# dimforge/salva

Hardware: AMD Instinct MI355X
Metric: particle-steps/sec (3D DFSPH) (higher is better)
Workload: dtype f32

## Files before the change

### salva_amd/csrc/device_types.h

```cpp
#pragma once
#include <hip/hip_runtime.h>

#include <cstdint>

#include "sph_math.h"

namespace salva {

struct TileGrid {
    int ox, oy, oz;
    int ntx, nty, ntz;
    uint32_t mx, my, mz;
    const uint32_t* cell_start;
};

struct TileAcc {
    uint64_t s;
    uint64_t sb;
    uint32_t nsl;
    uint32_t nonempty;
    uint32_t max_s, max_sb, max_nsl;
    uint32_t max_sum;
    uint32_t max_raw;
    uint32_t wsl;
    uint32_t ntiny;
    uint32_t heavy;
    uint32_t nlight;
    __host__ __device__ TileAcc operator+(const TileAcc& o) const {
        return TileAcc{s + o.s, sb + o.sb, nsl + o.nsl, nonempty + o.nonempty, max_s > o.max_s ? max_s : o.max_s,
                       max_sb > o.max_sb ? max_sb : o.max_sb, max_nsl > o.max_nsl ? max_nsl : o.max_nsl,
                       max_sum > o.max_sum ? max_sum : o.max_sum, max_raw > o.max_raw ? max_raw : o.max_raw, wsl + o.wsl, ntiny + o.ntiny, heavy + o.heavy, nlight + o.nlight};
    }
};

struct alignas(16) SolveCtl {
    uint32_t done;
    uint32_t iters;
    float err;
    uint32_t seq;
    float tol;
    uint32_t min_iter;
    uint32_t mode;
    uint32_t pad;
};
static_assert(sizeof(SolveCtl) == 32, "SolveCtl: two 16-byte halves");

struct TileListStats { uint32_t sum_ff, sum_fb, max_ff, max_fb, own_ff, own_fb, ref_s, ref_sb; };

struct PrePub { int32_t on, chained; int32_t bbox[6]; };

struct StepCtx {
    SphConsts sc;
    uint32_t xcd;

    uint32_t n;
    float4* posm;
    float4* vel;
    float4* dv;
    float4* acc;
    float4* w;
    float4* normal;
    uint32_t* model;
    uint32_t* perm;
    const uint32_t* gtag;
    float* rho;
    float* alpha;
    float* kappa;
    float* kappa2;
    float* rho_star;
    float* aii;
    float4* dii;
    float4* dijpj;
    float4* posmr;
    float4* iisph_q;
    float4* iisph_pr;
    uint32_t* nff;
    uint32_t* nfb;
    uint32_t* nbr_ff;
    uint32_t* nbr_fb;
    uint32_t* slice_near;
    uint32_t cap_ff, cap_fb;
    const TileAcc* tile_off;
    const uint32_t* halo_src;
    const uint32_t* bhalo_src;
    uint32_t halo_stride;
    uint32_t bhalo_stride;
    uint32_t ntiles;
    uint32_t split_s;
    const uint32_t* tile_ids;
    const uint4* slot_desc;
    const uint4* slot_info;
    const uint32_t* tile_rank;
    const uint32_t* slot_order;
    uint32_t slot_base;
    uint32_t ntiny;
    uint32_t nlight;
    uint32_t nlaunch;
    uint32_t spec;
    uint32_t halo_cap, bhalo_cap;
    uint32_t nslices_cap;
    uint64_t halo_len, bhalo_len;
    TileGrid gf;
    const uint32_t* stale_keys;

    uint32_t nb;
    float4* bposv;
    float4* bvel;
    uint32_t* bperm;
    float4* bforce;
    unsigned long long* bforce_fx;
    float bforce_scale;
    const uint8_t* bwants;
    TileGrid gb;

    uint32_t nmodels, nbmodels;
    const float* rho0_tab;
    float rho0_single;
    float mass_uniform;
    uint32_t* tile_mass_bits;
    uint32_t* tile_massb_bits;
    uint2* tile_masscd_bits;
    uint32_t* nffb;
    uint32_t* nffc;
    uint32_t two_mass;
    uint32_t nmass;
    uint64_t cmask;
    float class_mass[4];
    uint32_t bvel_zero;
    const uint8_t* ff_ok;
    const uint8_t* fb_ok;
    const uint8_t* bb_ok;

    float* partials;
    int spec_k;
    uint32_t spec_external;
    SolveCtl* spec_ring;
    SolveCtl* spec_pub;
    const uint32_t* model_counts;
    float4* w2;
    uint32_t* flags;
    uint32_t min_neighbors_for_divergence;
    int32_t phase, ghost_lo_cx, ghost_hi_cx;
    const SolveCtl* ctl;
    const uint32_t* gate;
    uint32_t gate_stage;
#ifdef SALVA_HIP_DIAG
    unsigned long long* dbg;
#endif
};

constexpr uint32_t MASS_SLOTS = 64;

struct Readback {
    float err;
    uint32_t flags;
    int32_t bbox[6];
    int32_t bbbox[6];
    TileAcc tile_total;
    uint64_t ncontacts_bb;
    uint64_t ncontacts_ff, ncontacts_fb;
    uint32_t max_cnt_ff, max_cnt_fb;
    uint32_t dcs_count;
    uint32_t cfl_max_bits;
    uint64_t ncontacts_own_ff, ncontacts_own_fb;
    uint32_t mass_mm[2];
    uint32_t pad2_[2];
    uint32_t chain_ok, chain_stage;
    uint32_t solve[2][4];
    uint32_t pre_ok;
    uint32_t max_ref[3];
};
// ... 7 lines not shown
```

### salva_amd/csrc/dfsph.hip

```cpp
#include <climits>

#include "bbox.h"
#include "kernels.h"
#include "tile.h"

namespace SALVA_KNS {
using namespace salva;

unsigned num_blocks(uint32_t n) { return div_up(n, BLOCK); }

}
#include "pairs.h"
namespace SALVA_KNS {
using namespace salva;

static inline bool plane_layouts(const StepCtx& c) { return c.mass_uniform > 0.0f || c.two_mass != 0u; }

#ifndef SALVA_DA_IISPH_WAVES
#define SALVA_DA_IISPH_WAVES 6
#endif
template <bool IISPH>
__global__ __launch_bounds__(TILE_MAX_THREADS, IISPH ? SALVA_DA_IISPH_WAVES : 1) void k_density_alpha(StepCtx c, float dt) {
    lds_base_check();
    Tile t;
    t.setup(c);
    if (t.empty()) return;
    struct Own { float4 pi; uint32_t mi, cnt; ListRegs lh; };
    auto load_own = [&](uint32_t i, uint32_t gs) { return Own{c.posm[i], c.model[i], c.nff[i], list_regs(c, gs)}; };
    uint32_t i0, gs0;
    t.first_own(i0, gs0);
    const Own own0 = load_own(i0, gs0);
    const float4* Lp = nullptr;
    t.stage(c, static_cast<const float4*>(c.posm), Lp);
    const float4* Bp = nullptr;
    t.stage_boundary(c, Bp);
    Tile::staged_barrier();
    t.for_own_pre(own0, load_own, [&](const Own& o, uint32_t i, uint32_t gs, bool active) {
        const uint32_t nqu = slice_list_dwords(o.cnt, active);
        const float4 pi = o.pi;
        float rho = 0.0f, gsx = 0.0f, gsy = 0.0f, gsz = 0.0f, sq = 0.0f;
        uint32_t nnear = 0;
        if (active) {
            f2 rw = {0.0f, 0.0f}, ax = {0.0f, 0.0f}, ay = {0.0f, 0.0f}, az = {0.0f, 0.0f}, s2 = {0.0f, 0.0f};
            const f2 tiny = {1.0e-30f, 1.0e-30f};
            for_each_ff2<true, false, true>(c, gs, nqu, o.lh, [&](uint32_t off) { return lds_ld16(off); }, [&](const float4& A, const float4& B) { SALVA_PAIR_MATH
                const f2 dx = {pi.x - A.x, pi.x - B.x}, dy = {pi.y - A.y, pi.y - B.y}, dz = {pi.z - A.z, pi.z - B.z};
                f2 r2 = dz * dz + tiny;
                r2 = dy * dy + r2;
                r2 = dx * dx + r2;
                const bool za = r2.x <= c.sc.tiny_r2, zb = r2.y <= c.sc.tiny_r2;
                nnear += (za ? 1u : 0u) + (zb ? 1u : 0u);
                const KernelWG2 k = kernel_wg2(r2, c.sc);
                const f2 m = {A.w, B.w};
                f2 wm = k.w * m;
                wm.x = za ? 0.0f : wm.x; wm.y = zb ? 0.0f : wm.y;
                rw += wm;
                const f2 gm = k.g * m;
                ax += dx * gm; ay += dy * gm; az += dz * gm;
                if (!IISPH) s2 += (gm * gm) * r2;
                else s2 += (k.g * gm) * r2;
            });
            const uint32_t npad = 2u * nqu - o.cnt;
            rho = (rw.x + rw.y) * c.sc.wscale + pi.w * c.sc.wnorm;
            gsx = (ax.x + ax.y) * c.sc.gscale; gsy = (ay.x + ay.y) * c.sc.gscale; gsz = (az.x + az.y) * c.sc.gscale;
            sq = (s2.x + s2.y) * (c.sc.gscale * c.sc.gscale);
            nnear -= npad;
        }
#ifdef SALVA_OTHER_KERNELS
        const bool any_near = __builtin_amdgcn_ballot_w64(active && nnear > 1u) != 0ull || (c.sc.kd | c.sc.kg) != 0;
#else
        const bool any_near = __builtin_amdgcn_ballot_w64(active && nnear > 1u) != 0ull;
#endif
        if (any_near && active) {
            rho = gsx = gsy = gsz = sq = 0.0f;
            for_each_ff(c, i, gs, [&](uint32_t s) { SALVA_PAIR_MATH
                const float4 pj = lds_ld16(s << 4);
                const float dx = pi.x - pj.x, dy = pi.y - pj.y, dz = pi.z - pj.z;
                const KernelEval e = kernel_eval(dx * dx + dy * dy + dz * dz, c.sc);
                rho += pj.w * e.w;
                const float gm = e.g * pj.w;
                const float gx = dx * gm, gy = dy * gm, gz = dz * gm;
                if (!IISPH) sq += gx * gx + gy * gy + gz * gz;
// ... 234 lines not shown
template <uint32_t DS>
__global__ __launch_bounds__(TILE_MAX_THREADS) void k_divergence(StepCtx c) {
    const SolveCtl* const rec = solve_record(c);
    if (rec && rec->done) return;
    const float4* const win = rec ? solve_w_in(c, rec) : c.w;
    lds_base_check();
    Tile t;
    t.setup(c);
    if (t.skipped()) return;
    if (t.empty()) { TileErr::zero(c, t.slot); return; }
    struct Own { float4 pi, wi; float alpha; uint32_t mi, cnt, cntb, near; ListRegs lh; };
    auto load_own = [&](uint32_t i, uint32_t gs) {
        return Own{c.posm[i], win[i], c.alpha[i], c.model[i], c.nff[i], c.nb ? c.nfb[i] : 0u, c.slice_near[gs], list_regs(c, gs)};
    };
    uint32_t i0, gs0;
    t.first_own(i0, gs0);
    const Own own0 = load_own(i0, gs0);
    const uint32_t dist = pw_dist<DS>(c, t);
    const float4* Bp = nullptr;
    const float4* Bv = nullptr;
    t.stage_pw(c, static_cast<const float4*>(c.posm), win, dist, Bp, Bv, false);
    TileErr E;
    E.init(carve_errtab(t), c);
    Tile::staged_barrier();
    t.for_own_pre(own0, load_own, [&](const Own& o, uint32_t i, uint32_t gs, bool active) {
        const uint32_t nqu = slice_list_dwords(o.cnt, active);
        const bool near = slice_is_near(c, o.near);
        float err = 0.0f;
        uint32_t mi = 0;
        if (active) {
            mi = o.mi;
            const float rho0 = rho0_of(c, mi);
            float div = 0.0f;
            if (o.cnt + o.cntb >= c.min_neighbors_for_divergence) {
                const float4 pi = o.pi, wi = o.wi;
                div += near ? pair_sum_velocity_divergence_exact(c, i, gs, pi, wi, dist)
                            : pair_sum_velocity_divergence(c, gs, nqu, o.lh, pi, wi, dist);
                for_each_fb(c, t, i, gs, [&](uint32_t s) { SALVA_PAIR_MATH
                    const float4 pj = Bp[s];
                    const float dx = pi.x - pj.x, dy = pi.y - pj.y, dz = pi.z - pj.z;
                    const float g = kernel_grad(dx * dx + dy * dy + dz * dz, c.sc);
                    div += (wi.x * dx + wi.y * dy + wi.z * dz) * g * (pj.w * rho0);
                });
                div = fmaxf(div, 0.0f);
            }
            c.kappa[i] = div * o.alpha;
            err = div / rho0;
        }
        E.add(c, err, mi, active && !is_ghost(c, i));
    });
    E.finish(c, t.slot);
}
#define SALVA_P3_BOUNDS(DS) __launch_bounds__(TILE_MAX_THREADS, (DS) == P3_DS_THREE ? 6 : 5)
#ifndef SALVA_EVAL_POST
#define SALVA_EVAL_POST false
#endif
template <uint32_t DS, int TWO>
__device__ __forceinline__ void k_divergence_p3_body(StepCtx c) {
    const SolveCtl* const rec = solve_record(c);
    if (rec && rec->done) return;
    const float4* const win = rec ? solve_w_in(c, rec) : c.w;
    lds_base_check();
    Tile t;
    t.setup(c);
    if (t.skipped()) return;
    if (t.empty()) { TileErr::zero(c, t.slot); return; }
    constexpr bool POST = TWO || SALVA_EVAL_POST;
    struct Own { float px, py, pz, ux, uy, uz, alpha; uint32_t mi, cnt, cntb, nb2, near; ListRegs lh; };
    auto load_own = [&](uint32_t i, uint32_t gs) {
        const float4 p = c.posm[i], u = win[i];
        return Own{p.x, p.y, p.z, u.x, u.y, u.z, POST ? 0.0f : c.alpha[i], POST ? 0u : c.model[i], c.nff[i], c.nb ? c.nfb[i] : 0u,
                   (TWO && t.massb != 0.0f) ? c.nffb[i] : 0u, c.slice_near[gs], list_regs(c, gs)};
    };
    uint32_t i0, gs0;
    t.first_own(i0, gs0);
    const Own own0 = load_own(i0, gs0);
    const uint32_t dist8 = p3_dist8<DS>(t);
    t.stage_p3(c, static_cast<const float4*>(c.posm), win, dist8);
    const float4* Bp = nullptr;
    t.stage_boundary(c, Bp);
    TileErrC E;
    E.init(reinterpret_cast<float*>(t.pool + t.pool_used), c);
    Tile::staged_barrier();
    t.for_own_pre(own0, load_own, [&](const Own& o, uint32_t i, uint32_t gs, bool active) {
        const uint32_t nqu = slice_list_dwords(o.cnt, active);
        const bool near = slice_is_near(c, o.near);
        float err = 0.0f;
        uint32_t mi = 0;
        if (active) {
            mi = POST ? c.model[i] : o.mi;
            const float rho0 = rho0_of(c, mi);
            float div = 0.0f;
            if (o.cnt + o.cntb >= c.min_neighbors_for_divergence) {
                const float4 pi = make_float4(o.px, o.py, o.pz, 0.0f), wi = make_float4(o.ux, o.uy, o.uz, 0.0f);
                if ((TWO && t.massb != 0.0f) && !near) {
                    div += pair_sum_velocity_divergence_p3_two(c, gs, nqu, o.lh, pi, wi, dist8, o.cnt - o.nb2, t.mass, t.massb);
                } else {
                    div += near ? pair_sum_velocity_divergence_exact_p3(c, i, gs, pi, wi, dist8, t.mass)
                                : pair_sum_velocity_divergence_p3(c, gs, nqu, o.lh, pi, wi, dist8, t.mass);
                    if ((TWO && t.massb != 0.0f) && o.nb2)
                        div += (t.massb - t.mass) * pair_tail_velocity_divergence_p3(c, gs, o.cnt - o.nb2, o.cnt, pi, wi, dist8);
                }
                if (TWO == 2 && t.massc != 0.0f) {
                    const uint32_t cd = c.nffc[i], l2 = cd & 0xffffu, l3 = cd >> 16;
                    if (l2) div += (t.massc - t.massb) * pair_tail_velocity_divergence_p3(c, gs, o.cnt - l3 - l2, o.cnt - l3, pi, wi, dist8);
                    if (l3) div += (t.massd - t.massb) * pair_tail_velocity_divergence_p3(c, gs, o.cnt - l3, o.cnt, pi, wi, dist8);
                }
                for_each_fb(c, t, i, gs, [&](uint32_t s) { SALVA_PAIR_MATH
                    const float4 pj = Bp[s];
                    const float dx = pi.x - pj.x, dy = pi.y - pj.y, dz = pi.z - pj.z;
                    const float g = kernel_grad(dx * dx + dy * dy + dz * dz, c.sc);
                    div += (wi.x * dx + wi.y * dy + wi.z * dz) * g * (pj.w * rho0);
                });
                div = fmaxf(div, 0.0f);
            }
            c.kappa[i] = div * (POST ? c.alpha[i] : o.alpha);
            err = div / rho0;
        }
        E.add(c, err, mi, active && !is_ghost(c, i));
    });
    E.finish(c, t.slot);
}
template <uint32_t DS>
__global__ SALVA_P3_BOUNDS(DS) void k_divergence_p3(StepCtx c) { k_divergence_p3_body<DS, 0>(c); }
template <uint32_t DS>
__global__ SALVA_P3_BOUNDS(DS) void k_divergence_p3_two(StepCtx c) { k_divergence_p3_body<DS, 1>(c); }
template <uint32_t DS>
__global__ SALVA_P3_BOUNDS(DS) void k_divergence_p3_multi(StepCtx c) { k_divergence_p3_body<DS, 2>(c); }
void launch_divergence(const StepCtx& c, const TileLds& L, hipStream_t s) {
    SALVA_OK_DISPATCH(launch_divergence, c, L, s);
    if (plane_layouts(c)) {
        const uint32_t ds = pick_ds_p3(L.max_halo_fluid, L.ds_level);
        if (c.two_mass && c.nmass > 2u) SALVA_LAUNCH_P3(k_divergence_p3_multi, ds, c, L, p3_bytes(L, ds, c.nmodels, false), s, c);
        else if (c.two_mass) SALVA_LAUNCH_P3(k_divergence_p3_two, ds, c, L, p3_bytes(L, ds, c.nmodels, false), s, c);
        else SALVA_LAUNCH_P3(k_divergence_p3, ds, c, L, p3_bytes(L, ds, c.nmodels, false), s, c);
        return;
    }
    const uint32_t ds = pick_ds(pw_slots(L), L.ds_level);
    SALVA_LAUNCH_FIXED(k_divergence, ds, c, L, pw_bytes(L, ds, true), s, c);
}

template <uint32_t DS>
__global__ __launch_bounds__(TILE_MAX_THREADS) void k_divergence_apply(StepCtx c, float inv_dt_prev) {
    const SolveCtl* const rec = solve_record(c);
    const bool was_done = rec && rec->done;
    const float4* const win = rec ? solve_w_in(c, rec) : c.w;
    float4* const wout = c.spec_k >= 0 ? ((win == c.w) ? c.w2 : c.w) : c.w;
    lds_base_check();
    if (c.spec_k >= 0 && !c.spec_external && blockIdx.x == 0 && c.slot_base == 0u) {
        spec_decide(c, reinterpret_cast<float*>(tile_smem));
        __syncthreads();
    }
    if (was_done) return;
    Tile t;
    t.setup(c);
    if (t.empty()) return;
    struct Own { float4 pi, wi; float ki; uint32_t cnt, near; ListRegs lh; };
    auto load_own = [&](uint32_t i, uint32_t gs) {
        return Own{c.posm[i], win[i], c.kappa[i], c.nff[i], c.slice_near[gs], list_regs(c, gs)};
    };
    uint32_t i0, gs0;
    t.first_own(i0, gs0);
    const Own own0 = load_own(i0, gs0);
    const uint32_t dist = pk_dist<DS>(c, t);
    const float4* Bp = nullptr;
    const float4* Bv = nullptr;
    t.stage_pk(c, static_cast<const float4*>(c.posm), static_cast<const float*>(c.kappa), dist, Bp, Bv);
    Tile::staged_barrier();
    t.for_own_pre(own0, load_own, [&](const Own& o, uint32_t i, uint32_t gs, bool active) {
        const uint32_t nqu = slice_list_dwords(o.cnt, active);
        const bool near = slice_is_near(c, o.near);
        if (!active) return;
        const float4 pi = o.pi;
        const uint32_t mi = __float_as_uint(o.wi.w);
        const float rho0 = rho0_of(c, mi);
        const float ki = o.ki;
        float4 d = o.wi;
        float sx, sy, sz;
        if (near) pair_sum_gradient_exact(c, i, gs, pi, dist, [&](float kj) { return ki + kj; }, sx, sy, sz);
        else pair_sum_gradient(c, gs, nqu, o.lh, pi, dist, [&](float ka, float kb) { return f2{ki + ka, ki + kb}; }, sx, sy, sz);
        d.x -= sx; d.y -= sy; d.z -= sz;
        for_each_fb(c, t, i, gs, [&](uint32_t s) { SALVA_PAIR_MATH
            const float4 pj = Bp[s];
            const float dx = pi.x - pj.x, dy = pi.y - pj.y, dz = pi.z - pj.z;
            const float g = kernel_grad(dx * dx + dy * dy + dz * dz, c.sc);
            const float coeff = -ki * pj.w * rho0 * g;
            const float ex = dx * coeff, ey = dy * coeff, ez = dz * coeff;
            d.x += ex; d.y += ey; d.z += ez;
            if (c.bforce && !is_ghost(c, i)) {
                const float fs = -inv_dt_prev * pi.w;
                apply_boundary_force(c, boundary_sorted_of_slot(c, t, s), __float_as_uint(Bv[s].w), ex * fs, ey * fs, ez * fs);
            }
        });
        wout[i] = d;
    });
}
#ifndef SALVA_P2_WAVES
#define SALVA_P2_WAVES 6
#endif
#define SALVA_P2_BOUNDS(DS) __launch_bounds__(TILE_MAX_THREADS, (DS) == P2_DS_THREE ? SALVA_P2_WAVES : 5)
template <uint32_t DS, int TWO>
__device__ __forceinline__ void k_divergence_apply_p2_body(StepCtx c, float inv_dt_prev) {
    const SolveCtl* const rec = solve_record(c);
    const bool was_done = rec && rec->done;
    const float4* const win = rec ? solve_w_in(c, rec) : c.w;
    float4* const wout = c.spec_k >= 0 ? ((win == c.w) ? c.w2 : c.w) : c.w;
    lds_base_check();
    if (c.spec_k >= 0 && !c.spec_external && blockIdx.x == 0 && c.slot_base == 0u) {
        spec_decide(c, reinterpret_cast<float*>(tile_smem));
        __syncthreads();
    }
    if (was_done) return;
    Tile t;
    t.setup(c);
    if (t.empty()) return;
    struct Own { float px, py, pz, ki; uint32_t cnt, nb2, near; ListRegs lh; };
    auto load_own = [&](uint32_t i, uint32_t gs) {
        const float4 p = c.posm[i];
        return Own{p.x, p.y, p.z, c.kappa[i], c.nff[i], (TWO && t.massb != 0.0f) ? c.nffb[i] : 0u, c.slice_near[gs], list_regs(c, gs)};
    };
    uint32_t i0, gs0;
    t.first_own(i0, gs0);
    const Own own0 = load_own(i0, gs0);
    const uint32_t dist8 = p2_dist8<DS>(t);
    t.stage_p2(c, static_cast<const float4*>(c.posm), static_cast<const float*>(c.kappa), dist8);
    Tile::staged_barrier();
    t.for_own_pre(own0, load_own, [&](const Own& o, uint32_t i, uint32_t gs, bool active) {
        const uint32_t nqu = slice_list_dwords(o.cnt, active);
        const bool near = slice_is_near(c, o.near);
        if (!active) return;
        const float4 pi = make_float4(o.px, o.py, o.pz, 0.0f);
        const float ki = o.ki;
        float sx, sy, sz;
        if ((TWO && t.massb != 0.0f) && !near) {
            pair_sum_gradient_p2_two(c, gs, nqu, o.lh, pi, dist8, o.cnt - o.nb2, t.mass, t.massb, [&](float ka, float kb) { return f2{ki + ka, ki + kb}; }, sx, sy, sz);
        } else {
            if (near) pair_sum_gradient_exact_p2(c, i, gs, pi, dist8, t.mass, [&](float kj) { return ki + kj; }, sx, sy, sz);
            else pair_sum_gradient_p2(c, gs, nqu, o.lh, pi, dist8, t.mass, [&](float ka, float kb) { return f2{ki + ka, ki + kb}; }, sx, sy, sz);
            if ((TWO && t.massb != 0.0f) && o.nb2) {
                float bx, by, bz;
                pair_tail_gradient_p2(c, gs, o.cnt - o.nb2, o.cnt, pi, dist8, [&](float kj) { return ki + kj; }, bx, by, bz);
                const float dm = t.massb - t.mass;
                sx += dm * bx; sy += dm * by; sz += dm * bz;
            }
        }
        if (TWO == 2 && t.massc != 0.0f) {
            const uint32_t cd = c.nffc[i], l2 = cd & 0xffffu, l3 = cd >> 16;
            float bx, by, bz;
            if (l2) {
                pair_tail_gradient_p2(c, gs, o.cnt - l3 - l2, o.cnt - l3, pi, dist8, [&](float kj) { return ki + kj; }, bx, by, bz);
                const float dm = t.massc - t.massb;
                sx += dm * bx; sy += dm * by; sz += dm * bz;
            }
            if (l3) {
                pair_tail_gradient_p2(c, gs, o.cnt - l3, o.cnt, pi, dist8, [&](float kj) { return ki + kj; }, bx, by, bz);
                const float dm = t.massd - t.massb;
                sx += dm * bx; sy += dm * by; sz += dm * bz;
            }
        }
        float4 d = win[i];
        const uint32_t mi = __float_as_uint(d.w);
        const float rho0 = rho0_of(c, mi);
        d.x -= sx; d.y -= sy; d.z -= sz;
        for_each_fb(c, t, i, gs, [&](uint32_t s) { SALVA_PAIR_MATH
            const float4 pj = p2_boundary_pos(t, s, dist8);
            const float dx = pi.x - pj.x, dy = pi.y - pj.y, dz = pi.z - pj.z;
            const float g = kernel_grad(dx * dx + dy * dy + dz * dz, c.sc);
            const float coeff = -ki * pj.w * rho0 * g;
            const float ex = dx * coeff, ey = dy * coeff, ez = dz * coeff;
            d.x += ex; d.y += ey; d.z += ez;
            if (c.bforce && !is_ghost(c, i)) {
                const float fs = -inv_dt_prev * c.posm[i].w;
                const uint32_t jb = boundary_sorted_of_slot(c, t, s);
                apply_boundary_force(c, jb, __float_as_uint(c.bvel[jb].w), ex * fs, ey * fs, ez * fs);
            }
        });
        wout[i] = d;
    });
}
template <uint32_t DS>
__global__ SALVA_P2_BOUNDS(DS) void k_divergence_apply_p2(StepCtx c, float inv_dt_prev) { k_divergence_apply_p2_body<DS, 0>(c, inv_dt_prev); }
template <uint32_t DS>
__global__ SALVA_P2_BOUNDS(DS) void k_divergence_apply_p2_two(StepCtx c, float inv_dt_prev) { k_divergence_apply_p2_body<DS, 1>(c, inv_dt_prev); }
template <uint32_t DS>
__global__ SALVA_P2_BOUNDS(DS) void k_divergence_apply_p2_multi(StepCtx c, float inv_dt_prev) { k_divergence_apply_p2_body<DS, 2>(c, inv_dt_prev); }
void launch_divergence_apply(const StepCtx& c, const TileLds& L, float inv_dt_prev, hipStream_t s) {
    SALVA_OK_DISPATCH(launch_divergence_apply, c, L, inv_dt_prev, s);
    if (plane_layouts(c)) {
        const uint32_t ds = pick_ds_p2(L.raw_slots(), L.ds_level);
        if (c.two_mass && c.nmass > 2u) SALVA_LAUNCH_P2(k_divergence_apply_p2_multi, ds, c, L, p2_bytes(L, ds), s, c, inv_dt_prev);
        else if (c.two_mass) SALVA_LAUNCH_P2(k_divergence_apply_p2_two, ds, c, L, p2_bytes(L, ds), s, c, inv_dt_prev);
        else SALVA_LAUNCH_P2(k_divergence_apply_p2, ds, c, L, p2_bytes(L, ds), s, c, inv_dt_prev);
        return;
    }
    const uint32_t ds = pick_ds(pk_slots(L), L.ds_level);
    SALVA_LAUNCH_FIXED(k_divergence_apply, ds, c, L, pk_bytes(L, ds), s, c, inv_dt_prev);
}

__global__ __launch_bounds__(BLOCK) void k_finish_divergence(StepCtx c, float gx, float gy, float gz, int acc_has_user) {
    const uint32_t i = blockIdx.x * BLOCK + threadIdx.x;
    if (i >= c.n || gate_closed(c)) return;
    const float4 wi = c.w[i];
    const float4 v = c.vel[i];
    const float4 d = c.dv[i];
    c.vel[i] = make_float4(wi.x, wi.y, wi.z, v.w);
    c.dv[i] = make_float4(0.0f, 0.0f, 0.0f, d.w);
    float4 a = make_float4(0.0f, 0.0f, 0.0f, 0.0f);
    if (acc_has_user) a = c.acc[i];
    c.acc[i] = make_float4(a.x + gx, a.y + gy, a.z + gz, 0.0f);
}
void launch_finish_divergence(const StepCtx& c, float gx, float gy, float gz, bool acc_has_user, hipStream_t s) {
    if (c.n) k_finish_divergence<<<num_blocks(c.n), BLOCK, 0, s>>>(c, gx, gy, gz, acc_has_user ? 1 : 0);
}

__global__ __launch_bounds__(BLOCK) void k_integrate(StepCtx c, float dt) {
    const uint32_t i = blockIdx.x * BLOCK + threadIdx.x;
    if (i >= c.n || gate_closed(c)) return;
    const float4 a = c.acc[i];
    float4 d = c.dv[i];
    d.x += a.x * dt; d.y += a.y * dt; d.z += a.z * dt;
    c.dv[i] = d;
    c.acc[i] = make_float4(0.0f, 0.0f, 0.0f, 0.0f);
    const float4 v = c.vel[i];
    c.w[i] = make_float4(v.x + d.x, v.y + d.y, v.z + d.z, __uint_as_float(c.model[i]));
}
void launch_integrate(const StepCtx& c, float dt, hipStream_t s) {
    if (c.n) k_integrate<<<num_blocks(c.n), BLOCK, 0, s>>>(c, dt);
}

#ifdef SALVA_HIP_DIAG
#define SALVA_DIAG_STAMP(name) const unsigned long long name = __builtin_readcyclecounter()
#else
#define SALVA_DIAG_STAMP(name)
#endif
template <uint32_t DS>
__global__ __launch_bounds__(TILE_MAX_THREADS) void k_pred_density(StepCtx c, float dt) {
    if (c.ctl && c.ctl->done) return;
    lds_base_check();
    SALVA_DIAG_STAMP(T0);
    Tile t;
    t.setup(c);
    if (t.skipped()) return;
    if (t.empty()) { TileErr::zero(c, t.slot); return; }
    SALVA_DIAG_STAMP(T1);
    struct Own { float4 pi, wi; float rho, alpha; uint32_t mi, cnt, near; ListRegs lh; };
    auto load_own = [&](uint32_t i, uint32_t gs) {
        return Own{c.posm[i], c.w[i], c.rho[i], c.alpha[i], c.model[i], c.nff[i], c.slice_near[gs], list_regs(c, gs)};
    };
    uint32_t i0, gs0;
    t.first_own(i0, gs0);
    const Own own0 = load_own(i0, gs0);
    const uint32_t dist = pw_dist<DS>(c, t);
    const float4* Bp = nullptr;
    const float4* Bv = nullptr;
    t.stage_pw(c, static_cast<const float4*>(c.posm), static_cast<const float4*>(c.w), dist, Bp, Bv, true);
    TileErr E;
    E.init(carve_errtab(t), c);
    SALVA_DIAG_STAMP(T2);
    Tile::staged_barrier();
    SALVA_DIAG_STAMP(T3);
    t.for_own_pre(own0, load_own, [&](const Own& o, uint32_t i, uint32_t gs, bool active) {
// ... 437 lines not shown
```

### salva_amd/csrc/pairs.h

```cpp
#pragma once
#include <cstdlib>

#include "tile.h"

namespace salva {

struct RecPW { float4 p, w; };
struct RecPK { float4 p; float k; };

__device__ __forceinline__ float rho0_of(const StepCtx& c, uint32_t model) {
    return (c.nmodels == 1) ? c.rho0_single : c.rho0_tab[model];
}

template <uint32_t DS>
__device__ __forceinline__ uint32_t pw_dist(const StepCtx& c, const Tile& t) { return DS ? DS * 16u : (t.stage_cap(c) + t.SB) * 16u; }
template <uint32_t DS>
__device__ __forceinline__ uint32_t pk_dist(const StepCtx& c, const Tile& t) { return DS ? DS * 16u : (t.stage_cap(c) + 2u * t.SB) * 16u; }

__device__ __forceinline__ RecPW load_pw(uint32_t o, uint32_t dist) {
    RecPW r{lds_ld16(o), lds_ld16(o + dist)};
    asm volatile("" ::"v"(r.w.w));
    return r;
}
__device__ __forceinline__ RecPK load_pk(uint32_t o, uint32_t dist) { return RecPK{lds_ld16(o), lds_ld4((o >> 2) + dist)}; }

template <bool AHEAD = true>
__device__ __forceinline__ float pair_sum_velocity_divergence(const StepCtx& c, uint32_t gs, uint32_t nqu, const ListRegs& lh,
                                                              const float4& pi, const float4& wi, uint32_t dist) {
    f2 acc2 = {0.0f, 0.0f};
    const f2 tiny = {1.0e-30f, 1.0e-30f};
    for_each_ff2<AHEAD, false, true>(c, gs, nqu, lh, [&](uint32_t o) { return load_pw(o, dist);
    }, [&](const RecPW& A, const RecPW& B) { SALVA_PAIR_MATH
        const f2 dx = {pi.x - A.p.x, pi.x - B.p.x}, dy = {pi.y - A.p.y, pi.y - B.p.y}, dz = {pi.z - A.p.z, pi.z - B.p.z};
        f2 r2 = dz * dz + tiny;
        r2 = dy * dy + r2;
        r2 = dx * dx + r2;
        const f2 g = kernel_gfac2(r2, c.sc);
        const f2 ux = {wi.x - A.w.x, wi.x - B.w.x}, uy = {wi.y - A.w.y, wi.y - B.w.y}, uz = {wi.z - A.w.z, wi.z - B.w.z};
        const f2 gm = {g.x * A.p.w, g.y * B.p.w};
        acc2 += (ux * dx + uy * dy + uz * dz) * gm;
    });
    return (acc2.x + acc2.y) * c.sc.gscale;
}
__device__ __forceinline__ float pair_sum_velocity_divergence_exact(const StepCtx& c, uint32_t i, uint32_t gs, const float4& pi,
                                                                    const float4& wi, uint32_t dist) {
    float acc = 0.0f;
    for_each_ff(c, i, gs, [&](uint32_t s) { SALVA_PAIR_MATH
        const RecPW A = load_pw(s << 4, dist);
        const float dx = pi.x - A.p.x, dy = pi.y - A.p.y, dz = pi.z - A.p.z;
        const float g = kernel_grad(dx * dx + dy * dy + dz * dz, c.sc);
        acc += ((wi.x - A.w.x) * dx + (wi.y - A.w.y) * dy + (wi.z - A.w.z) * dz) * g * A.p.w;
    });
    return acc;
}
struct RecP3 { lds_v2f xy, zu, vw; };
template <uint32_t DS>
__device__ __forceinline__ uint32_t p3_dist8(const Tile& t) { return DS ? DS * 8u : ((t.S * 8u + 15u) & ~15u); }
template <uint32_t DS>
__device__ __forceinline__ uint32_t p2_dist8(const Tile& t) { return DS ? DS * 8u : (((t.S + t.SB) * 8u + 15u) & ~15u); }
__device__ __forceinline__ RecP3 load_p3(uint32_t o, uint32_t dist8) { return RecP3{lds_ld8(o), lds_ld8(o + dist8), lds_ld8(o + 2u * dist8)}; }
template <bool AHEAD = true>
__device__ __forceinline__ float pair_sum_velocity_divergence_p3(const StepCtx& c, uint32_t gs, uint32_t nqu, const ListRegs& lh,
                                                                 const float4& pi, const float4& wi, uint32_t dist8, float mass) {
    f2 acc2 = {0.0f, 0.0f};
    const f2 tiny = {1.0e-30f, 1.0e-30f};
    for_each_ff2<AHEAD, false, 2>(c, gs, nqu, lh, [&](uint32_t o) { return load_p3(o, dist8); }, [&](const RecP3& A, const RecP3& B) { SALVA_PAIR_MATH
        const f2 dx = {pi.x - A.xy.x, pi.x - B.xy.x}, dy = {pi.y - A.xy.y, pi.y - B.xy.y}, dz = {pi.z - A.zu.x, pi.z - B.zu.x};
        f2 r2 = dz * dz + tiny;
        r2 = dy * dy + r2;
        r2 = dx * dx + r2;
        const f2 g = kernel_gfac2(r2, c.sc);
        const f2 ux = {wi.x - A.zu.y, wi.x - B.zu.y}, uy = {wi.y - A.vw.x, wi.y - B.vw.x}, uz = {wi.z - A.vw.y, wi.z - B.vw.y};
        acc2 += (ux * dx + uy * dy + uz * dz) * g;
    });
    return (acc2.x + acc2.y) * c.sc.gscale * mass;
}
__device__ __forceinline__ float pair_sum_velocity_divergence_p3_two(const StepCtx& c, uint32_t gs, uint32_t nqu, const ListRegs& lh, const float4& pi,
                                                                     const float4& wi, uint32_t dist8, uint32_t na, float ma, float mb) {
    f2 acc2 = {0.0f, 0.0f};
    const f2 tiny = {1.0e-30f, 1.0e-30f};
    for_each_ff2_indexed<2>(c, gs, nqu, lh, [&](uint32_t o) { return load_p3(o, dist8); }, [&](const RecP3& A, const RecP3& B, uint32_t q) { SALVA_PAIR_MATH
        const f2 dx = {pi.x - A.xy.x, pi.x - B.xy.x}, dy = {pi.y - A.xy.y, pi.y - B.xy.y}, dz = {pi.z - A.zu.x, pi.z - B.zu.x};
        f2 r2 = dz * dz + tiny;
        r2 = dy * dy + r2;
        r2 = dx * dx + r2;
        const f2 g = kernel_gfac2(r2, c.sc);
        const f2 ux = {wi.x - A.zu.y, wi.x - B.zu.y}, uy = {wi.y - A.vw.x, wi.y - B.vw.x}, uz = {wi.z - A.vw.y, wi.z - B.vw.y};
        const f2 m = {2u * q < na ? ma : mb, 2u * q + 1u < na ? ma : mb};
        acc2 += (ux * dx + uy * dy + uz * dz) * (g * m);
    });
    return (acc2.x + acc2.y) * c.sc.gscale;
}
__device__ __forceinline__ float pair_sum_velocity_divergence_exact_p3(const StepCtx& c, uint32_t i, uint32_t gs, const float4& pi,
                                                                       const float4& wi, uint32_t dist8, float mass) {
    float acc = 0.0f;
    for_each_ff(c, i, gs, [&](uint32_t s) { SALVA_PAIR_MATH
        const RecP3 A = load_p3(s << 3, dist8);
        const float dx = pi.x - A.xy.x, dy = pi.y - A.xy.y, dz = pi.z - A.zu.x;
        const float g = kernel_grad(dx * dx + dy * dy + dz * dz, c.sc);
        acc += ((wi.x - A.zu.y) * dx + (wi.y - A.vw.x) * dy + (wi.z - A.vw.y) * dz) * g;
    });
    return acc * mass;
}
template <typename F>
__device__ __forceinline__ void for_each_ff_range(const StepCtx& c, uint32_t gs, uint32_t first, uint32_t cnt, F&& f) {
    const uint32_t* __restrict__ p = c.nbr_ff + (size_t)gs * c.cap_ff * WAVE + 4u * (threadIdx.x & (WAVE - 1));
    for (uint32_t e = first; e < cnt; ++e) {
        const uint32_t d = p[ellq(e >> 1)];
        f((e & 1u) ? (d >> 16) : (d & 0xffffu));
    }
}
__device__ __forceinline__ float pair_tail_velocity_divergence_p3(const StepCtx& c, uint32_t gs, uint32_t first, uint32_t cnt, const float4& pi,
                                                                  const float4& wi, uint32_t dist8) {
    float acc = 0.0f;
    for_each_ff_range(c, gs, first, cnt, [&](uint32_t s) { SALVA_PAIR_MATH
        const RecP3 A = load_p3(s << 3, dist8);
        const float dx = pi.x - A.xy.x, dy = pi.y - A.xy.y, dz = pi.z - A.zu.x;
        const float g = kernel_grad(dx * dx + dy * dy + dz * dz, c.sc);
        acc += ((wi.x - A.zu.y) * dx + (wi.y - A.vw.x) * dy + (wi.z - A.vw.y) * dz) * g;
    });
    return acc;
}
struct RecP2 { lds_v2f xy, zk; };
__device__ __forceinline__ RecP2 load_p2(uint32_t o, uint32_t dist8) { return RecP2{lds_ld8(o), lds_ld8(o + dist8)}; }
#ifndef SALVA_P2_NARROW
#define SALVA_P2_NARROW false
#endif
template <typename K2>
__device__ __forceinline__ void pair_sum_gradient_p2(const StepCtx& c, uint32_t gs, uint32_t nqu, const ListRegs& lh, const float4& pi,
                                                     uint32_t dist8, float mass, K2&& kij2, float& sx, float& sy, float& sz) {
    f2 ax = {0.0f, 0.0f}, ay = {0.0f, 0.0f}, az = {0.0f, 0.0f};
    const f2 tiny = {1.0e-30f, 1.0e-30f};
    for_each_ff2<true, false, 2, SALVA_P2_NARROW>(c, gs, nqu, lh, [&](uint32_t o) { return load_p2(o, dist8); }, [&](const RecP2& A, const RecP2& B) { SALVA_PAIR_MATH
        const f2 dx = {pi.x - A.xy.x, pi.x - B.xy.x}, dy = {pi.y - A.xy.y, pi.y - B.xy.y}, dz = {pi.z - A.zk.x, pi.z - B.zk.x};
        f2 r2 = dz * dz + tiny;
        r2 = dy * dy + r2;
        r2 = dx * dx + r2;
        const f2 g = kernel_gfac2(r2, c.sc);
        const f2 coeff = kij2(A.zk.y, B.zk.y) * g;
        ax += dx * coeff; ay += dy * coeff; az += dz * coeff;
    });
    const float f = c.sc.gscale * mass;
    sx = (ax.x + ax.y) * f; sy = (ay.x + ay.y) * f; sz = (az.x + az.y) * f;
}
template <typename K2>
__device__ __forceinline__ void pair_sum_gradient_p2_two(const StepCtx& c, uint32_t gs, uint32_t nqu, const ListRegs& lh, const float4& pi,
                                                         uint32_t dist8, uint32_t na, float ma, float mb, K2&& kij2, float& sx, float& sy, float& sz) {
    f2 ax = {0.0f, 0.0f}, ay = {0.0f, 0.0f}, az = {0.0f, 0.0f};
    const f2 tiny = {1.0e-30f, 1.0e-30f};
    for_each_ff2_indexed<2>(c, gs, nqu, lh, [&](uint32_t o) { return load_p2(o, dist8); }, [&](const RecP2& A, const RecP2& B, uint32_t q) { SALVA_PAIR_MATH
        const f2 dx = {pi.x - A.xy.x, pi.x - B.xy.x}, dy = {pi.y - A.xy.y, pi.y - B.xy.y}, dz = {pi.z - A.zk.x, pi.z - B.zk.x};
        f2 r2 = dz * dz + tiny;
        r2 = dy * dy + r2;
        r2 = dx * dx + r2;
        const f2 g = kernel_gfac2(r2, c.sc);
        const f2 m = {2u * q < na ? ma : mb, 2u * q + 1u < na ? ma : mb};
        const f2 coeff = kij2(A.zk.y, B.zk.y) * (g * m);
        ax += dx * coeff; ay += dy * coeff; az += dz * coeff;
    });
    sx = (ax.x + ax.y) * c.sc.gscale; sy = (ay.x + ay.y) * c.sc.gscale; sz = (az.x + az.y) * c.sc.gscale;
}
template <typename K1>
__device__ __forceinline__ void pair_sum_gradient_exact_p2(const StepCtx& c, uint32_t i, uint32_t gs, const float4& pi, uint32_t dist8,
                                                           float mass, K1&& kij1, float& sx, float& sy, float& sz) {
    float ax = 0.0f, ay = 0.0f, az = 0.0f;
    for_each_ff(c, i, gs, [&](uint32_t s) { SALVA_PAIR_MATH
        const RecP2 A = load_p2(s << 3, dist8);
        const float dx = pi.x - A.xy.x, dy = pi.y - A.xy.y, dz = pi.z - A.zk.x;
        const float coeff = kij1(A.zk.y) * kernel_grad(dx * dx + dy * dy + dz * dz, c.sc);
        ax += dx * coeff; ay += dy * coeff; az += dz * coeff;
    });
    sx = ax * mass; sy = ay * mass; sz = az * mass;
}
template <typename K1>
__device__ __forceinline__ void pair_tail_gradient_p2(const StepCtx& c, uint32_t gs, uint32_t first, uint32_t cnt, const float4& pi, uint32_t dist8,
                                                      K1&& kij1, float& sx, float& sy, float& sz) {
    float ax = 0.0f, ay = 0.0f, az = 0.0f;
    for_each_ff_range(c, gs, first, cnt, [&](uint32_t s) { SALVA_PAIR_MATH
        const RecP2 A = load_p2(s << 3, dist8);
        const float dx = pi.x - A.xy.x, dy = pi.y - A.xy.y, dz = pi.z - A.zk.x;
        const float coeff = kij1(A.zk.y) * kernel_grad(dx * dx + dy * dy + dz * dz, c.sc);
        ax += dx * coeff; ay += dy * coeff; az += dz * coeff;
    });
    sx = ax; sy = ay; sz = az;
}
__device__ __forceinline__ float4 p2_boundary_pos(const Tile& t, uint32_t s, uint32_t dist8) {
    const uint32_t o = (t.S + s) * 8u;
    const lds_v2f xy = lds_ld8(o), zv = lds_ld8(o + dist8);
    return make_float4(xy.x, xy.y, zv.x, zv.y);
}
static inline uint32_t p2_bytes(const TileLds& L, uint32_t ds) {
    const uint32_t n = L.raw_slots();
    const uint32_t dist8 = ds ? ds * 8u : ((n * 8u + 15u) & ~15u);
    return dist8 + n * 8u + 32u;
}

template <typename K2>
__device__ __forceinline__ void pair_sum_gradient(const StepCtx& c, uint32_t gs, uint32_t nqu, const ListRegs& lh, const float4& pi,
                                                  uint32_t dist, K2&& kij2, float& sx, float& sy, float& sz) {
    f2 ax = {0.0f, 0.0f}, ay = {0.0f, 0.0f}, az = {0.0f, 0.0f};
    const f2 tiny = {1.0e-30f, 1.0e-30f};
    for_each_ff2<true, false, true>(c, gs, nqu, lh, [&](uint32_t o) { return load_pk(o, dist); }, [&](const RecPK& A, const RecPK& B) { SALVA_PAIR_MATH
        const f2 dx = {pi.x - A.p.x, pi.x - B.p.x}, dy = {pi.y - A.p.y, pi.y - B.p.y}, dz = {pi.z - A.p.z, pi.z - B.p.z};
        f2 r2 = dz * dz + tiny;
        r2 = dy * dy + r2;
        r2 = dx * dx + r2;
        const f2 g = kernel_gfac2(r2, c.sc);
        const f2 km = kij2(A.k, B.k) * f2{A.p.w, B.p.w};
        const f2 coeff = km * g;
        ax += dx * coeff; ay += dy * coeff; az += dz * coeff;
    });
    sx = (ax.x + ax.y) * c.sc.gscale; sy = (ay.x + ay.y) * c.sc.gscale; sz = (az.x + az.y) * c.sc.gscale;
}
template <typename K1>
__device__ __forceinline__ void pair_sum_gradient_exact(const StepCtx& c, uint32_t i, uint32_t gs, const float4& pi, uint32_t dist,
                                                        K1&& kij1, float& sx, float& sy, float& sz) {
    float ax = 0.0f, ay = 0.0f, az = 0.0f;
    for_each_ff(c, i, gs, [&](uint32_t s) { SALVA_PAIR_MATH
        const RecPK A = load_pk(s << 4, dist);
        const float dx = pi.x - A.p.x, dy = pi.y - A.p.y, dz = pi.z - A.p.z;
        const float coeff = kij1(A.k) * A.p.w * kernel_grad(dx * dx + dy * dy + dz * dz, c.sc);
        ax += dx * coeff; ay += dy * coeff; az += dz * coeff;
    });
    sx = ax; sy = ay; sz = az;
}
__device__ __forceinline__ bool slice_is_near(const StepCtx& c, uint32_t near_word) {
#ifdef SALVA_OTHER_KERNELS
    return (__builtin_amdgcn_readfirstlane((int)near_word) | c.sc.kg) != 0;
#else
    return __builtin_amdgcn_readfirstlane((int)near_word) != 0;
#endif
}
__device__ __forceinline__ float (*carve_errtab(Tile& t))[MAX_MODELS] {
    return reinterpret_cast<float (*)[MAX_MODELS]>(t.carve<float>(TILE_MAX_WAVES * MAX_MODELS));
}

#define SALVA_LAUNCH_FIXED(kernel, DSV, c, L, lds, s, ...)                                                         \
    do {                                                                                                           \
        if ((DSV) == FIXED_DS_SMALL) SALVA_LAUNCH_TILE_3(kernel<FIXED_DS_SMALL>, kernel<FIXED_DS_SMALL>, FIXED_DS_SMALL, kernel<0u>, c, L, lds, s, __VA_ARGS__); \
        else if ((DSV) == FIXED_DS_LARGE) SALVA_LAUNCH_TILE_3(kernel<FIXED_DS_LARGE>, kernel<FIXED_DS_SMALL>, FIXED_DS_SMALL, kernel<0u>, c, L, lds, s, __VA_ARGS__); \
        else SALVA_LAUNCH_TILE_3(kernel<0u>, kernel<FIXED_DS_SMALL>, FIXED_DS_SMALL, kernel<0u>, c, L, lds, s, __VA_ARGS__); \
    } while (0)
static inline uint32_t pick_ds(uint32_t slots_needed, uint32_t level) {
    const uint32_t ds[3] = {FIXED_DS_SMALL, FIXED_DS_LARGE, 0u};
    uint32_t k = slots_needed <= FIXED_DS_SMALL ? 0u : (slots_needed <= FIXED_DS_LARGE ? 1u : 2u);
    k += level;
    return ds[k < 2u ? k : 2u];
}
static inline uint32_t pw_slots(const TileLds& L) { return L.sum_slots(); }
static inline uint32_t pw_bytes(const TileLds& L, uint32_t ds, bool errtab) {
    return (ds ? 2u * ds : 2u * pw_slots(L)) * 16u + (errtab ? TILE_ERR_BYTES : 0u) + 32u;
}
static inline uint32_t pick_ds_p3(uint32_t s, uint32_t level) {
    const uint32_t ds[4] = {P3_DS_THREE, P3_DS_TWO, P3_DS_ONE, 0u};
    uint32_t k = s <= P3_DS_THREE ? 0u : (s <= P3_DS_TWO ? 1u : (s <= P3_DS_ONE ? 2u : 3u));
    k += level;
    return ds[k < 3u ? k : 3u];
}
static inline uint32_t p3_bytes(const TileLds& L, uint32_t ds, uint32_t nmodels, bool with_bv) {
    const uint32_t dist8 = ds ? ds * 8u : ((L.max_halo_fluid * 8u + 15u) & ~15u);
    const uint32_t bb = with_bv ? 32u : 16u;
    const uint32_t by_maxima = ((L.max_halo_fluid * 8u + 15u) & ~15u) + bb * L.max_halo_boundary;
    const uint32_t by_raw = ((L.raw_slots() * 8u + 15u) & ~15u) + (bb - 8u) * L.max_halo_boundary;
    static const uint32_t pad = getenv("SALVA_HIP_P3_PAD") ? (uint32_t)atoi(getenv("SALVA_HIP_P3_PAD")) : 0u;
    return 2u * dist8 + (by_raw < by_maxima ? by_raw : by_maxima) + ((TILE_MAX_WAVES * nmodels * 4u + 15u) & ~15u) + 32u + pad;
}
static inline uint32_t pick_ds_p2(uint32_t n, uint32_t level) {
    const uint32_t ds[4] = {P2_DS_THREE, P3_DS_TWO, P3_DS_ONE, 0u};
    uint32_t k = n <= P2_DS_THREE ? 0u : (n <= P3_DS_TWO ? 1u : (n <= P3_DS_ONE ? 2u : 3u));
    k += level;
    return ds[k < 3u ? k : 3u];
}
#define SALVA_LAUNCH_P3(kernel, DSV, c, L, lds, s, ...)                                                                                          \
    do {                                                                                                                                         \
        if ((DSV) == P3_DS_THREE) SALVA_LAUNCH_TILE_3(kernel<P3_DS_THREE>, kernel<P3_DS_THREE>, P3_DS_THREE, kernel<0u>, c, L, lds, s, __VA_ARGS__); \
        else if ((DSV) == P3_DS_TWO) SALVA_LAUNCH_TILE_3(kernel<P3_DS_TWO>, kernel<P3_DS_THREE>, P3_DS_THREE, kernel<0u>, c, L, lds, s, __VA_ARGS__); \
        else if ((DSV) == P3_DS_ONE) SALVA_LAUNCH_TILE_3(kernel<P3_DS_ONE>, kernel<P3_DS_THREE>, P3_DS_THREE, kernel<0u>, c, L, lds, s, __VA_ARGS__); \
        else SALVA_LAUNCH_TILE_3(kernel<0u>, kernel<P3_DS_THREE>, P3_DS_THREE, kernel<0u>, c, L, lds, s, __VA_ARGS__);                             \
    } while (0)
#define SALVA_LAUNCH_P2(kernel, DSV, c, L, lds, s, ...)                                                                                          \
    do {                                                                                                                                         \
        if ((DSV) == P2_DS_THREE) SALVA_LAUNCH_TILE_3(kernel<P2_DS_THREE>, kernel<P2_DS_THREE>, P2_DS_THREE, kernel<0u>, c, L, lds, s, __VA_ARGS__); \
        else if ((DSV) == P3_DS_TWO) SALVA_LAUNCH_TILE_3(kernel<P3_DS_TWO>, kernel<P2_DS_THREE>, P2_DS_THREE, kernel<0u>, c, L, lds, s, __VA_ARGS__); \
        else if ((DSV) == P3_DS_ONE) SALVA_LAUNCH_TILE_3(kernel<P3_DS_ONE>, kernel<P2_DS_THREE>, P2_DS_THREE, kernel<0u>, c, L, lds, s, __VA_ARGS__); \
        else SALVA_LAUNCH_TILE_3(kernel<0u>, kernel<P2_DS_THREE>, P2_DS_THREE, kernel<0u>, c, L, lds, s, __VA_ARGS__);                             \
    } while (0)
static inline uint32_t pk_slots(const TileLds& L) { return L.sum_slots() + L.max_halo_boundary; }
static inline uint32_t pk_bytes(const TileLds& L, uint32_t ds) {
    return (ds ? ds : pk_slots(L)) * 16u + ((L.max_halo_fluid + 63u) & ~63u) * 4u + 32u;
}


}
```

### salva_amd/csrc/tile.h

```cpp
#pragma once
#include "common.h"
#include "device_types.h"

namespace salva {

#ifndef SALVA_TX
#define SALVA_TX 4
#endif
constexpr int TX = SALVA_TX, TY = 4, TZ = 4;
constexpr int TCELLS = TX * TY * TZ;
constexpr int HX = TX + 2, HY = TY + 2, HZ = TZ + 2;
constexpr int HCELLS = HX * HY * HZ;
constexpr int TILE_MAX_WAVES = 12;
constexpr int TILE_MAX_THREADS = TILE_MAX_WAVES * WAVE;

__host__ __device__ inline int floor_div(int a, int b) { return (a >= 0) ? a / b : -((-a + b - 1) / b); }

__host__ __device__ inline uint32_t ellq(uint32_t q) { return (q >> 2) * (4u * (uint32_t)WAVE) + (q & 3u); }

constexpr uint32_t TILE_TABLE_BYTES = 4 * (2 * (HCELLS + 1) + 2 * HCELLS) + 16;

struct TileLds {
    uint32_t max_halo_fluid = 0, max_halo_boundary = 0, threads = 4 * WAVE;
    uint32_t max_sum = 0;
    uint32_t max_raw = 0;
    uint32_t ds_level = 0;
    uint32_t raw_slots() const { return max_raw ? max_raw : max_halo_fluid + max_halo_boundary; }
    uint32_t sum_slots() const {
        const uint32_t worst = ((max_halo_fluid + 63u) & ~63u) + max_halo_boundary;
        return max_sum ? (max_sum < worst ? max_sum : worst) : worst;
    }
    uint32_t bytes(uint32_t bytes_per_fluid_slot, uint32_t bytes_per_boundary_slot, uint32_t narrays,
                   bool with_cell_tables = false) const {
        const uint32_t separate = ((max_halo_fluid + 63u) & ~63u) * bytes_per_fluid_slot + max_halo_boundary * bytes_per_boundary_slot;
        const uint32_t wide = bytes_per_fluid_slot > bytes_per_boundary_slot ? bytes_per_fluid_slot : bytes_per_boundary_slot;
        const uint32_t joint = sum_slots() * wide;
        return (with_cell_tables ? TILE_TABLE_BYTES : 0u) + (joint < separate ? joint : separate) + 16u * narrays;
    }
};

#ifndef SALVA_FIXED_DS_SMALL
#define SALVA_FIXED_DS_SMALL 2448
#endif
constexpr uint32_t FIXED_DS_SMALL = SALVA_FIXED_DS_SMALL, FIXED_DS_LARGE = 3984;
#ifndef SALVA_P3_DS3
#define SALVA_P3_DS3 2080
#endif
constexpr uint32_t P3_DS_THREE = SALVA_P3_DS3, P3_DS_TWO = 3360, P3_DS_ONE = 4064;
#ifndef SALVA_P2_DS3
#define SALVA_P2_DS3 2464
#endif
constexpr uint32_t P2_DS_THREE = SALVA_P2_DS3;
static_assert((P3_DS_THREE % 64 == 32 && P3_DS_TWO % 64 == 32 && P3_DS_ONE % 64 == 32 && P2_DS_THREE % 64 == 32) || SALVA_P3_DS3 != 2080 || SALVA_P2_DS3 != 2464,
              "plane distances: odd multiples of 256 bytes");
constexpr uint32_t TILE_PART_SHIFT = 28;
constexpr uint32_t TILE_PART_WHOLE = (uint32_t)(TX - 1) << 2;
__host__ __device__ inline uint32_t tile_part_code(uint32_t ux0, uint32_t len) { return ux0 | ((len - 1u) << 2); }
constexpr uint32_t TILE_SPLIT_S = P3_DS_THREE;
constexpr uint32_t TILE_TINY_S = 192, TILE_TINY_SB = 64, TILE_TINY_THREADS = 64;
constexpr uint32_t TILE_ERR_BYTES = 12u * 32u * 4u;

#ifdef __HIPCC__

void raise_tile_lds_limit(const void* kernel, uint32_t bytes);
template <typename K>
inline void ensure_tile_lds(K kernel, uint32_t bytes) {
    if (bytes > 48u * 1024u) raise_tile_lds_limit(reinterpret_cast<const void*>(kernel), bytes);
}
inline TileLds tile_tiny_lds(const TileLds& L) {
    TileLds t = L;
    t.max_halo_fluid = TILE_TINY_S; t.max_halo_boundary = L.max_halo_boundary ? TILE_TINY_SB : 0u;
    t.max_sum = ((TILE_TINY_S + 63u) & ~63u) + t.max_halo_boundary; t.max_raw = TILE_TINY_S + t.max_halo_boundary;
    t.threads = TILE_TINY_THREADS;
    return t;
}
__host__ __device__ inline bool tile_is_light(uint32_t s, uint32_t sb) {
    return s <= P3_DS_THREE && ((s + 63u) & ~63u) + 2u * sb <= FIXED_DS_SMALL;
}
inline TileLds tile_light_lds(const TileLds& L) {
    TileLds t = L;
    t.max_halo_fluid = L.max_halo_fluid < P3_DS_THREE ? L.max_halo_fluid : P3_DS_THREE;
    t.max_halo_boundary = L.max_halo_boundary < FIXED_DS_SMALL / 2u ? L.max_halo_boundary : FIXED_DS_SMALL / 2u;
    t.max_sum = (L.max_sum && L.max_sum < FIXED_DS_SMALL) ? L.max_sum : FIXED_DS_SMALL;
    t.max_raw = (L.max_raw && L.max_raw < FIXED_DS_SMALL) ? L.max_raw : FIXED_DS_SMALL;
    return t;
}
#define SALVA_LAUNCH_TILE_3(kernel, kernel_light, ds_light, kernel_tiny, c, L, lds, s, ...)         \
    do {                                                                                           \
        if ((c).n && (c).nlaunch) {                                                                \
            if (((c).ntiny == 0u && (c).nlight == 0u) || (c).slot_order == nullptr) {              \
                const uint32_t _lds = (lds);                                                       \
                ::salva::ensure_tile_lds(kernel, _lds);                                            \
                kernel<<<(c).nlaunch, (L).threads, _lds, s>>>(__VA_ARGS__);                        \
            } else {                                                                               \
                const uint32_t _ntiny = (c).ntiny, _nlight = (c).nlight;                           \
                const uint32_t _nfull = (c).nlaunch - _nlight - _ntiny;                            \
                ::salva::StepCtx _c2 = (c);                                                        \
                const ::salva::TileLds _lt = ::salva::tile_tiny_lds(L);                            \
                const ::salva::TileLds _ll = ::salva::tile_light_lds(L);                           \
                const unsigned _thr = (L).threads;                                                 \
                if (_nfull) {                                                                      \
                    const uint32_t _lds = (lds);                                                   \
                    ::salva::ensure_tile_lds(kernel, _lds);                                        \
                    _c2.slot_base = 0u;                                                            \
                    { const ::salva::StepCtx c = _c2; kernel<<<_nfull, _thr, _lds, s>>>(__VA_ARGS__); } \
                }                                                                                  \
                if (_nlight) {                                                                     \
                    _c2.slot_base = _nfull;                                                        \
                    const ::salva::TileLds L = _ll;                                                \
                    const uint32_t ds = (ds_light); (void)ds;                                      \
                    const ::salva::StepCtx c = _c2;                                                \
                    const uint32_t _lds = (lds);                                                   \
                    ::salva::ensure_tile_lds(kernel_light, _lds);                                  \
                    kernel_light<<<_nlight, _thr, _lds, s>>>(__VA_ARGS__);                         \
                }                                                                                  \
                if (_ntiny) {                                                                      \
                    _c2.slot_base = _nfull + _nlight;                                              \
                    const ::salva::TileLds L = _lt;                                                \
                    const uint32_t ds = 0u; (void)ds;                                              \
                    const ::salva::StepCtx c = _c2;                                                \
                    const uint32_t _lds = (lds);                                                   \
                    ::salva::ensure_tile_lds(kernel_tiny, _lds);                                   \
                    kernel_tiny<<<_ntiny, TILE_TINY_THREADS, _lds, s>>>(__VA_ARGS__);              \
                }                                                                                  \
            }                                                                                      \
            SALVA_HIP_CHECK(hipGetLastError());                                                    \
        }                                                                                          \
    } while (0)
#define SALVA_LAUNCH_TILE(kernel, c, L, lds, s, ...) SALVA_LAUNCH_TILE_3(kernel, kernel, 0u, kernel, c, L, lds, s, __VA_ARGS__)

__device__ __forceinline__ uint32_t tile_key_m(const TileGrid& g, int cx, int cy, int cz, bool& inside, uint32_t mx, uint32_t my, uint32_t mz) {
    const uint32_t ix = ((uint32_t)cx - (uint32_t)g.ox) & mx, iy = ((uint32_t)cy - (uint32_t)g.oy) & my, iz = ((uint32_t)cz - (uint32_t)g.oz) & mz;
    inside = ix < (uint32_t)(g.ntx * TX) && iy < (uint32_t)(g.nty * TY) && iz < (uint32_t)(g.ntz * TZ);
    const uint32_t tile = ((ix / TX) * (uint32_t)g.nty + (iy / TY)) * (uint32_t)g.ntz + (iz / TZ);
    return tile * TCELLS + (((ix % TX) * TY + (iy % TY)) * TZ + (iz % TZ));
}
__device__ __forceinline__ uint32_t tile_key(const TileGrid& g, int cx, int cy, int cz, bool& inside) {
    return tile_key_m(g, cx, cy, cz, inside, g.mx, g.my, g.mz);
}

__device__ __forceinline__ int cell_coord(float x, float h, bool& bad) {
    float f = floorf(__fdiv_rn(x, h));
// ... 273 lines not shown
        if (c.halo_stride) {
            const uint32_t pre[PRE] = {pre0, pre1, pre2, pre3};
            float4 a[PRE], b[PRE];
#pragma unroll
            for (int k = 0; k < PRE; ++k) {
                const uint32_t sl = s0 + (uint32_t)k * nt;
                const uint32_t g = sl < S ? pre[k] : own_begin;
                a[k] = posm[g]; b[k] = w[g];
            }
#pragma unroll
            for (int k = 0; k < PRE; ++k) {
                const uint32_t sl = s0 + (uint32_t)k * nt;
                if (sl < S) p3_store(sl, dist8, a[k], b[k]);
            }
            for (uint32_t sl = s0 + PRE * nt; sl < S; sl += nt) {
                const uint32_t g = c.halo_src[hoff + sl];
                p3_store(sl, dist8, posm[g], w[g]);
            }
        } else {
            for_halo(c, [&](uint32_t sl, uint32_t g) { p3_store(sl, dist8, posm[g], w[g]); });
        }
        pool_used = 2u * dist8 + ((S * 8u + 15u) & ~15u);
    }
    __device__ __forceinline__ void stage_p2(const StepCtx& c, const float4* __restrict__ posm, const float* __restrict__ k, uint32_t dist8) {
        const uint32_t nt = blockDim.x, s0 = threadIdx.x;
        if (c.halo_stride) {
            const uint32_t pre[PRE] = {pre0, pre1, pre2, pre3};
            float4 a[PRE];
            float b[PRE];
#pragma unroll
            for (int q = 0; q < PRE; ++q) {
                const uint32_t sl = s0 + (uint32_t)q * nt;
                const uint32_t g = sl < S ? pre[q] : own_begin;
                a[q] = posm[g]; b[q] = k[g];
            }
#pragma unroll
            for (int q = 0; q < PRE; ++q) {
                const uint32_t sl = s0 + (uint32_t)q * nt;
                if (sl < S) { lds_st8(sl * 8u, a[q].x, a[q].y); lds_st8(sl * 8u + dist8, a[q].z, b[q]); }
            }
            for (uint32_t sl = s0 + PRE * nt; sl < S; sl += nt) {
                const uint32_t g = c.halo_src[hoff + sl];
                const float4 p = posm[g];
                lds_st8(sl * 8u, p.x, p.y); lds_st8(sl * 8u + dist8, p.z, k[g]);
            }
        } else {
            for_halo(c, [&](uint32_t sl, uint32_t g) {
                const float4 p = posm[g];
                lds_st8(sl * 8u, p.x, p.y); lds_st8(sl * 8u + dist8, p.z, k[g]);
            });
        }
        for_halo_boundary(c, [&](uint32_t sl, uint32_t g) {
            const float4 p = c.bposv[g];
            lds_st8((S + sl) * 8u, p.x, p.y); lds_st8((S + sl) * 8u + dist8, p.z, p.w);
        });
        pool_used = dist8 + (S + SB) * 8u;
    }
    static __device__ __forceinline__ void staged_barrier() {
        asm volatile("s_waitcnt vmcnt(0)" ::: "memory");
        __syncthreads();
    }
    __device__ __forceinline__ void stage_boundary(const StepCtx& c, const float4*& bp) {
        float4* a = carve<float4>(SB);
        for_halo_boundary(c, [&](uint32_t s, uint32_t g) { a[s] = c.bposv[g]; });
        bp = a;
    }
    __device__ __forceinline__ void stage_boundary(const StepCtx& c, const float4*& bp, const float4*& bv) {
        float4* a = carve<float4>(SB); float4* b = carve<float4>(SB);
        for_halo_boundary(c, [&](uint32_t s, uint32_t g) { a[s] = c.bposv[g]; b[s] = c.bvel[g]; });
        bp = a; bv = b;
    }

    __device__ __forceinline__ bool first_own(uint32_t& i, uint32_t& gs) const {
        const uint32_t s = threadIdx.x / WAVE, nsl = (own_end - own_begin + WAVE - 1) / WAVE;
        i = own_begin + s * WAVE + (threadIdx.x & (WAVE - 1));
        gs = slice_base + s;
        const bool ok = s < nsl && i < own_end;
        if (!ok) { i = own_begin; gs = slice_base; }
        return ok;
    }
    template <typename Pre, typename LoadOwn, typename Body>
    __device__ __forceinline__ void for_own_pre(const Pre& pre0, LoadOwn&& load_own, Body&& body) const {
        const uint32_t nsl = (own_end - own_begin + WAVE - 1) / WAVE;
        const uint32_t lane = threadIdx.x & (WAVE - 1), nw = blockDim.x / WAVE;
        uint32_t s = threadIdx.x / WAVE;
        if (s < nsl) {
            const uint32_t i = own_begin + s * WAVE + lane;
            body(pre0, i, slice_base + s, i < own_end);
            s += nw;
        }
        for (; s < nsl; s += nw) {
            const uint32_t i = own_begin + s * WAVE + lane, gs = slice_base + s;
            const bool active = i < own_end;
            const Pre p = load_own(active ? i : own_begin, gs);
            body(p, i, gs, active);
        }
    }

    template <typename F>
    __device__ __forceinline__ void for_own(F&& f) const {
        const uint32_t nsl = (own_end - own_begin + WAVE - 1) / WAVE;
        const uint32_t lane = threadIdx.x & (WAVE - 1), nw = blockDim.x / WAVE;
        for (uint32_t s = threadIdx.x / WAVE; s < nsl; s += nw) {
            const uint32_t i = own_begin + s * WAVE + lane;
            f(i, slice_base + s, i < own_end);
        }
    }
};

struct TileCells {
    uint32_t *lstart, *gstart, *blstart, *bgstart;

    __device__ __forceinline__ void build(const StepCtx& c, Tile& t, bool clamp_to_staged = false) {
        uint32_t* tab = t.carve<uint32_t>(2 * (HCELLS + 1) + 2 * HCELLS);
        lstart = tab; gstart = tab + (HCELLS + 1); blstart = gstart + HCELLS; bgstart = blstart + (HCELLS + 1);
        for (int h = threadIdx.x; h < HCELLS; h += blockDim.x) {
            const int hz = h % HZ, hy = (h / HZ) % HY, hx = h / (HZ * HY);
            const bool plane = (uint32_t)hx >= t.part_ux0() && (uint32_t)hx < t.part_ux0() + t.part_len() + 2u;
            bool in;
            const uint32_t k = tile_key(c.gf, t.hcx + hx, t.hcy + hy, t.hcz + hz, in);
            uint32_t b = 0, e = 0;
            if (in && plane) { b = c.gf.cell_start[k]; e = c.gf.cell_start[k + 1]; }
            gstart[h] = b; lstart[h] = e - b;
            b = e = 0;
            if (c.nb && plane) {
                const uint32_t kb = tile_key_m(c.gb, t.hcx + hx, t.hcy + hy, t.hcz + hz, in, c.gf.mx, c.gf.my, c.gf.mz);
                if (in) { b = c.gb.cell_start[kb]; e = c.gb.cell_start[kb + 1]; }
            }
            bgstart[h] = b; blstart[h] = e - b;
        }
        __syncthreads();
        if (threadIdx.x < WAVE) {
            constexpr int PER = (HCELLS + WAVE - 1) / WAVE;
            constexpr int NL = (HCELLS + PER - 1) / PER;
            const int l = threadIdx.x;
            uint32_t a[PER], b[PER], sa = 0, sb = 0;
#pragma unroll
            for (int k = 0; k < PER; ++k) {
                const bool in = PER * l + k < HCELLS;
                a[k] = in ? lstart[PER * l + k] : 0u;
                b[k] = in ? blstart[PER * l + k] : 0u;
                sa += a[k]; sb += b[k];
            }
            uint32_t ia = sa, ib = sb;
#pragma unroll
            for (int o = 1; o < WAVE; o <<= 1) {
                const uint32_t ta = (uint32_t)__shfl_up((int)ia, o, WAVE), tb = (uint32_t)__shfl_up((int)ib, o, WAVE);
                if (l >= o) { ia += ta; ib += tb; }
            }
            uint32_t ea = ia - sa, eb = ib - sb;
            if (l < NL) {
#pragma unroll
                for (int k = 0; k < PER; ++k) {
                    if (PER * l + k < HCELLS) { lstart[PER * l + k] = ea; blstart[PER * l + k] = eb; }
                    ea += a[k]; eb += b[k];
                }
            }
            if (l == NL - 1) { lstart[HCELLS] = ia; blstart[HCELLS] = ib; }
        }
        __syncthreads();
        if (clamp_to_staged && c.spec) {
            for (int q = threadIdx.x; q <= HCELLS; q += blockDim.x) {
                lstart[q] = min(lstart[q], t.S);
                blstart[q] = min(blstart[q], t.SB);
            }
            __syncthreads();
        }
    }
};

template <typename L, typename C>
__device__ __forceinline__ void for_each_slot(const uint32_t* __restrict__ nbr, uint32_t cap, uint32_t gslice,
                                              uint32_t cnt, L&& load, C&& compute) {
    if (cnt == 0) return;
    const uint32_t* __restrict__ p = nbr + (size_t)gslice * cap * WAVE + 4u * (threadIdx.x & (WAVE - 1));
    const uint32_t nq = (cnt + 1) >> 1;
    uint32_t q = 0;
    uint32_t n0 = p[0], n1 = (nq > 1) ? p[ellq(1)] : 0u;
    for (; q + 2 <= nq; q += 2) {
// ... 130 lines not shown
                compute2(d0, d1);
            }
        }
    } else {
#pragma unroll
    for (int k = 0; k < LIST_REGS; k += 2) {
        if (FUSED) {
            if ((uint32_t)(k + 1) < nq) {
                const uint32_t a = lr.d[k], b = lr.d[k + 1];
                const auto d0 = load(entry_lo<OFF>(a));
                const auto d1 = load(entry_hi<OFF>(a));
                const auto d2 = load(entry_lo<OFF>(b));
                const auto d3 = load(entry_hi<OFF>(b));
                compute2(d0, d1);
                compute2(d2, d3);
            } else if ((uint32_t)k < nq) {
                const uint32_t a = lr.d[k];
                const auto d0 = load(entry_lo<OFF>(a));
                const auto d1 = load(entry_hi<OFF>(a));
                compute2(d0, d1);
            }
        } else if ((uint32_t)k < nq) {
            const uint32_t a = lr.d[k];
            const bool two = (uint32_t)(k + 1) < nq;
            const uint32_t b = two ? lr.d[k + 1] : a;
            const auto d0 = load(entry_lo<OFF>(a));
            const auto d1 = load(entry_hi<OFF>(a));
            const auto d2 = load(entry_lo<OFF>(b));
            const auto d3 = load(entry_hi<OFF>(b));
            compute2(d0, d1);
            if (two) compute2(d2, d3);
        }
    }
    }
    if (nq > (uint32_t)LIST_REGS) {
        const uint32_t* __restrict__ p = c.nbr_ff + (size_t)gslice * c.cap_ff * WAVE + 4u * (threadIdx.x & (WAVE - 1));
        if (AHEAD) {
            uint32_t nx = p[ellq(LIST_REGS)];
            for (uint32_t q = LIST_REGS; q < nq; ++q) {
                const uint32_t a = nx;
                if (q + 1 < nq) nx = p[ellq(q + 1)];
                const auto d0 = load(entry_lo<OFF>(a));
                const auto d1 = load(entry_hi<OFF>(a));
                compute2(d0, d1);
            }
        } else {
            for (uint32_t q = LIST_REGS; q < nq; ++q) {
                const uint32_t a = p[ellq(q)];
                const auto d0 = load(entry_lo<OFF>(a));
                const auto d1 = load(entry_hi<OFF>(a));
                compute2(d0, d1);
            }
        }
    }
}
template <int OFF, typename L, typename C2>
__device__ __forceinline__ void for_each_ff2_indexed(const StepCtx& c, uint32_t gslice, uint32_t nq, const ListRegs& lr, L&& load, C2&& compute2) {
#pragma unroll
    for (int k = 0; k < LIST_REGS; k += 2) {
        if ((uint32_t)k < nq) {
            const uint32_t a = lr.d[k];
            const bool two = (uint32_t)(k + 1) < nq;
            const uint32_t b = two ? lr.d[k + 1] : a;
            const auto d0 = load(entry_lo<OFF>(a));
            const auto d1 = load(entry_hi<OFF>(a));
            const auto d2 = load(entry_lo<OFF>(b));
            const auto d3 = load(entry_hi<OFF>(b));
            compute2(d0, d1, (uint32_t)k);
            if (two) compute2(d2, d3, (uint32_t)(k + 1));
        }
    }
    if (nq > (uint32_t)LIST_REGS) {
        const uint32_t* __restrict__ p = c.nbr_ff + (size_t)gslice * c.cap_ff * WAVE + 4u * (threadIdx.x & (WAVE - 1));
        uint32_t nx = p[ellq(LIST_REGS)];
        for (uint32_t q = LIST_REGS; q < nq; ++q) {
            const uint32_t a = nx;
            if (q + 1 < nq) nx = p[ellq(q + 1)];
            const auto d0 = load(entry_lo<OFF>(a));
            const auto d1 = load(entry_hi<OFF>(a));
            compute2(d0, d1, q);
        }
    }
}
constexpr int FB_REGS = 8;
struct FbRegs { uint32_t d[FB_REGS]; };
__device__ __forceinline__ FbRegs fb_regs(const StepCtx& c, uint32_t gslice) {
    const uint32_t* __restrict__ p = (c.nb ? c.nbr_fb + (size_t)gslice * c.cap_fb * WAVE : c.nbr_ff + (size_t)gslice * c.cap_ff * WAVE) +
                                     4u * (threadIdx.x & (WAVE - 1));
    static_assert(FB_REGS % 4 == 0, "fetched in 16-byte pieces");
    const uint4* __restrict__ p4 = reinterpret_cast<const uint4*>(p);
    FbRegs r;
#pragma unroll
    for (int k = 0; k < FB_REGS / 4; ++k) {
        const uint4 v = p4[(size_t)k * WAVE];
        r.d[4 * k] = v.x; r.d[4 * k + 1] = v.y; r.d[4 * k + 2] = v.z; r.d[4 * k + 3] = v.w;
    }
    return r;
}
template <typename F>
__device__ __forceinline__ void for_each_fb_regs(const StepCtx& c, uint32_t SB, uint32_t gslice, uint32_t cnt, const FbRegs& fr, F&& f) {
    if (SB == 0 || cnt == 0) return;
    const uint32_t nq = (cnt + 1) >> 1;
#pragma unroll
    for (int k = 0; k < FB_REGS; ++k) {
        if ((uint32_t)k < nq) {
            const uint32_t a = fr.d[k];
            f(a & 0xffffu);
            if (2u * (uint32_t)k + 1u < cnt) f(a >> 16);
        }
    }
    if (nq > (uint32_t)FB_REGS) {
        const uint32_t* __restrict__ p = c.nbr_fb + (size_t)gslice * c.cap_fb * WAVE + 4u * (threadIdx.x & (WAVE - 1));
        for (uint32_t q = FB_REGS; q < nq; ++q) {
            const uint32_t a = p[ellq(q)];
            f(a & 0xffffu);
            if (2u * q + 1u < cnt) f(a >> 16);
        }
    }
}
struct ListOwn { uint32_t cnt; ListRegs lr; };
__device__ __forceinline__ ListOwn list_own(const StepCtx& c, uint32_t i, uint32_t gslice) { return ListOwn{c.nff[i], list_regs(c, gslice)}; }
template <typename L, typename C>
__device__ __forceinline__ void for_each_ff_regs(const StepCtx& c, uint32_t gslice, const ListOwn& o, L&& load, C&& compute) {
    const uint32_t cnt = o.cnt;
#pragma unroll
    for (int k = 0; k < LIST_REGS; ++k) {
        if (2u * (uint32_t)k < cnt) {
            const uint32_t a = o.lr.d[k];
            const auto d0 = load(a & 0xffffu);
            const auto d1 = load(a >> 16);
            compute(d0);
            if (2u * (uint32_t)k + 1u < cnt) compute(d1);
        }
    }
    if (cnt > 2u * (uint32_t)LIST_REGS) {
        const uint32_t* __restrict__ p = c.nbr_ff + (size_t)gslice * c.cap_ff * WAVE + 4u * (threadIdx.x & (WAVE - 1));
        const uint32_t nq = (cnt + 1u) >> 1;
        uint32_t nx = p[ellq(LIST_REGS)];
        for (uint32_t q = LIST_REGS; q < nq; ++q) {
            const uint32_t a = nx;
            if (q + 1 < nq) nx = p[ellq(q + 1)];
            const auto d0 = load(a & 0xffffu);
            const auto d1 = load(a >> 16);
            compute(d0);
            if (2u * q + 1u < cnt) compute(d1);
        }
    }
}
template <typename F>
__device__ __forceinline__ void for_each_ff_regs(const StepCtx& c, uint32_t gslice, const ListOwn& o, F&& f) {
    for_each_ff_regs(c, gslice, o, [](uint32_t s) { return s; }, f);
}
__device__ __forceinline__ uint32_t slice_list_dwords(uint32_t cnt, bool active) {
    return (uint32_t)__builtin_amdgcn_readfirstlane((int)wave_max_u32(active ? ((cnt + 1) >> 1) : 0u));
}
template <typename L, typename C>
__device__ __forceinline__ void for_each_ff(const StepCtx& c, uint32_t i, uint32_t gslice, L&& load, C&& compute) {
    for_each_slot(c.nbr_ff, c.cap_ff, gslice, c.nff[i], load, compute);
}
template <typename F>
__device__ __forceinline__ void for_each_ff(const StepCtx& c, uint32_t i, uint32_t gslice, F&& f) {
    for_each_slot(c.nbr_ff, c.cap_ff, gslice, c.nff[i], [](uint32_t s) { return s; }, f);
}
template <typename F>
__device__ __forceinline__ void for_each_fb(const StepCtx& c, const Tile& t, uint32_t i, uint32_t gslice, F&& f) {
    if (t.SB == 0) return;
// ... 84 lines not shown
```

### salva_amd/csrc/world.h

```cpp
#pragma once
#include <string>
#include <map>
#include <memory>
#include <vector>

#include "../../include/salva_hip.h"
#include "common.h"
#include "device_types.h"
#include "comm.h"
#include "dist.h"
#include "kernels.h"
#include "elastic.h"

namespace salva {

struct FluidSlot {
    uint64_t n = 0;
    float density0 = 1000.0f;
    float vol_uniform = 0.0f;
    uint32_t memberships = 1u, filter = 0xffffffffu;
    std::vector<SalvaHipForceDesc> forces;
    std::vector<uint32_t> force_iters;
    std::vector<float> force_errs;
    std::vector<std::shared_ptr<ElasticState>> elastic;
// ... 233 lines not shown
    uint32_t nmass = 0;
    float mass_classes[4] = {0.0f, 0.0f, 0.0f, 0.0f};
    uint64_t mass_cmask = 0;
    bool decide_two_mass();
    std::vector<hipEvent_t> dist_ev;
    size_t dist_ev_used = 0;
    std::vector<std::pair<size_t, int>> dist_ev_pairs;
    double dist_times[4] = {0.0, 0.0, 0.0, 0.0};
    size_t dist_time_begin(int kind);
    void dist_time_end(size_t first);
    void dist_time_fold();
    bool fused_first_divergence = false;
    bool flags_clean = false;
    bool check_mass = true;
    bool mass_known = false;
    bool tile_trace = false;
    bool no_fused_div = false;
    bool no_planes = false;
    bool iisph_dii_fused = false;
    int sort_mode = -1;
#ifdef SALVA_HIP_DIAG
    PipeCfg pipe;
#endif
    TileAcc pred_tt{};
    uint32_t pred_n = 0;
    bool pred_valid = false, spec_mode = false;
    uint32_t halo_cap = 0xffffffffu, bhalo_cap = 0xffffffffu, nslices_cap = 0xffffffffu;
    uint64_t halo_len = ~0ull, bhalo_len = ~0ull;
    uint64_t spec_misses = 0;
    bool trust_cap0 = false;
    bool lists_checked = false;
    bool defer_off = false;
    bool spec_off = true, spec_tight = false;
    int num_cus = 256;
    DevBuf<char> cub_temp;
    DevBuf<float> scratch_f;
    DevBuf<float4> scratch_f4;

    DevBuf<float4> bst_pos, bst_vel;
    DevBuf<float4> bposv, bvel, bforce;
    DevBuf<unsigned long long> bforce_fx;
    uint32_t bforce_fx_n = 0;
    float bforce_scale() const;
    DevBuf<uint32_t> bperm, cell_start_b, bkeys[2], bidx[2];
    bool b_dirty = true;
    uint64_t ncontacts_bb = 0;

    GridDims gf, gb;
    bool bbox_known = false;

    DevBuf<float> rho0_tab;
    DevBuf<uint8_t> ff_ok, fb_ok, bb_ok, bwants;
    DevBuf<uint32_t> model_counts;
    bool tables_dirty = true, any_wants_forces = false;

    DevBuf<float> partials;
    DevBuf<Readback> d_rb;
    DevBuf<uint32_t> mass_slots;
    struct FlagsPtr { uint32_t* p = nullptr; } d_flags;
    DevBuf<unsigned long long> d_counters;
    Readback* h_rb = nullptr;
    struct HostPub { uint32_t seq, pad[3]; Readback rb; };
    HostPub* h_hostpub = nullptr;
    uint32_t hostpub_seq = 0;
    uint32_t publish_enqueue(const TileAcc* totals, bool lists, bool end_of_step, const PrePub* pre = nullptr, const uint32_t* gate = nullptr);
    struct PreGrid {
        bool valid = false;
        uint32_t n = 0, seq = 0, nslots_bound = 0, ntiles = 0;
        size_t ncf = 0;
        bool check_mass = false;
        uint32_t split_s = 0;
        GridDims gf;
    } pre;
    bool pre_off = false;
    DevBuf<uint32_t> slot_order;
    DevBuf<unsigned int> hq_cnt;
    DevBuf<uint32_t> hq_kind, hq_index;
    DevBuf<float4> hq_pos;
    uint32_t hq_need = 0;
    uint32_t class_ntiny = 0;
    uint32_t class_nlight = 0;
    bool classes_off = false, classes_forced = false, light_on = false;
    bool split_off = false;
    bool ref_off = false, ref_forced = false;
    bool ref_tight = false;
    bool ref_on_cur = false;
    bool ref_bounded = false;
    bool ref_pred_valid = false;
    uint32_t ref_pred[3] = {0, 0, 0}, ref_pred_n = 0;
    bool ref_last = false;
    RefCaps ref_last_caps{0xffffffffu, 0xffffffffu, 0xffffffffu};
    TileLds lds_full;
    uint32_t ref_last_nslots_bound = 0;
    uint64_t ref_passes = 0, ref_misses = 0;
    uint32_t split_forced = 0;
    bool split_on = false;
    uint32_t split_s_cur = 0;
    int32_t bbox_used_last[6] = {0, 0, 0, 0, 0, 0};
    bool bbox_used_valid = false;
    uint64_t pre_adopted = 0, pre_dropped = 0;
    void pre_enqueue_grid(uint32_t nslots_bound);
    void pre_drop();
    void publish_wait(uint32_t seq, bool totals, bool lists, bool end_of_step);
    bool fold_stats = false;
    uint32_t fold_bbox_blocks = 0;
    const uint32_t* fold_bbox_gate = nullptr;
    void publish_and_wait(const TileAcc* totals, bool lists, bool end_of_step);
    DevBuf<SolveCtl> d_ctl;
    SolveCtl* h_ctl = nullptr;
    SolveCtl* h_pub = nullptr;

    struct StickyBuf { std::shared_ptr<DevBuf<float4>> data; uint64_t len = 0; };
    std::map<uint32_t, StickyBuf> sticky;
    SalvaHipForceCallback force_cb = nullptr;
    void* force_user = nullptr;
    SalvaHipWorld* force_owner = nullptr;
    bool in_force_cb = false;
    SalvaHipCouplingCallback coupling_cb = nullptr;
    void* coupling_user = nullptr;
    SalvaHipWorld* coupling_owner = nullptr;
    void call_coupling(int phase, float dt);
    float dt_prev = 0.0f, inv_dt_prev = 0.0f;
    StepCtx last_ctx{};
    float last_dt = 0.0f;
    bool have_last_ctx = false;
    hipEvent_t ev[3] = {nullptr, nullptr, nullptr};
    hipEvent_t evc[5] = {nullptr, nullptr, nullptr, nullptr, nullptr};
    uint64_t spec_passes = 0;
    hipEvent_t ev_sync = nullptr;

    Transport* comm = nullptr;
    int slab_lo = 0, slab_hi = 0;
    int nbr_lo_lo = INT32_MIN, nbr_hi_hi = INT32_MAX;
    bool nbr_bounds_valid = false;
    DevBuf<unsigned long long> plane_hist;
    std::vector<uint32_t> global_counts;
    uint32_t gid_offset = 0, n_owned = 0;
    uint64_t gid_next = 0;
    void dist_add_particles(uint32_t slot, uint64_t n_add, const float* pos, const float* vel_h);
    void dist_update_counts(const std::vector<long long>& delta);
    bool dist_started = false;
    DevBuf<uint32_t> gtag[2];
    DevBuf<DistRec> xsend_lo, xsend_hi, xrecv_lo, xrecv_hi;
    DevBuf<char> dsel, dpos;
    DevBuf<uint32_t> send_lo_idx, send_hi_idx, ghost_lo_idx, ghost_hi_idx;
    uint32_t nborder_lo = 0, nborder_hi = 0, nghost_lo = 0, nghost_hi = 0;
    DevBuf<float4> fbuf_send, fbuf_recv;
    DevBuf<float> d_sums;
};

}
```

### salva_amd/csrc/world.hip

```cpp
#include "world.h"
#include "dcs.h"
#include "bbox.h"

#include <algorithm>
#include <cfloat>
#include <cstddef>
#include <chrono>
#include <cmath>
#include <cstring>
#include <limits>

#include <mutex>
#include <unordered_map>

namespace salva {

void raise_tile_lds_limit(const void* kernel, uint32_t bytes) {
    if (bytes > 160u * 1024u)
        throw HipError(SALVA_HIP_E_CAPACITY, "a tile's halo does not fit the 160 KiB LDS (particles are compressed far beyond rest density)");
    static std::mutex mu;
    static std::unordered_map<const void*, uint32_t> granted;
    std::lock_guard<std::mutex> lock(mu);
    uint32_t& g = granted[kernel];
    if (bytes <= g) return;
// ... 32 lines not shown
    if (keep_w) v.w = dst[i].w;
    dst[i] = v;
}
__global__ void k_fill_w(uint32_t n, float4* __restrict__ dst, float v) {
    const uint32_t i = blockIdx.x * BLOCK + threadIdx.x;
    if (i < n) reinterpret_cast<float*>(&dst[i])[3] = v;
}
__global__ void k_fill_u32(uint32_t n, uint32_t* __restrict__ dst, uint32_t v) {
    const uint32_t i = blockIdx.x * BLOCK + threadIdx.x;
    if (i < n) dst[i] = v;
}
__global__ void k_unpack_xyz(uint32_t n, const float4* __restrict__ src, float* __restrict__ dst) {
    const uint32_t i = blockIdx.x * BLOCK + threadIdx.x;
    if (i >= n) return;
    const float4 s = src[i];
    dst[3 * i] = s.x; dst[3 * i + 1] = s.y; dst[3 * i + 2] = s.z;
}
__global__ void k_unpack_w(uint32_t n, const float4* __restrict__ src, float* __restrict__ dst) {
    const uint32_t i = blockIdx.x * BLOCK + threadIdx.x;
    if (i < n) dst[i] = src[i].w;
}
__global__ void k_set_bmodel(uint32_t n, float4* __restrict__ bvel, uint32_t m) {
    const uint32_t i = blockIdx.x * BLOCK + threadIdx.x;
    if (i < n) reinterpret_cast<float*>(&bvel[i])[3] = __uint_as_float(m);
}

static inline unsigned nblk(uint64_t n) { return div_up(n ? n : 1, BLOCK); }

struct Piece { uint64_t src_off, len; bool from_old; };

template <typename T>
static void rebuild(DevBuf<T>& buf, const std::vector<Piece>& pieces, uint64_t new_total, hipStream_t s) {
    DevBuf<T> nb;
    nb.ensure(new_total ? new_total : 1);
    uint64_t off = 0;
    for (const Piece& p : pieces) {
        if (p.from_old && p.len)
            SALVA_HIP_CHECK(hipMemcpyAsync(nb.p + off, buf.p + p.src_off, p.len * sizeof(T), hipMemcpyDeviceToDevice, s));
        off += p.len;
    }
    SALVA_HIP_CHECK(hipStreamSynchronize(s));
    std::swap(buf.p, nb.p);
    std::swap(buf.cap, nb.cap);
}

static int bits_for(uint64_t ncells) {
    int b = 1;
    while (b < 32 && ((uint64_t)1 << b) < ncells) ++b;
    return b;
}

World::World(const SalvaHipParams& p) : prm(p) {
    if (!(p.particle_radius > 0.0f) || !(p.smoothing_factor > 0.0f))
        throw HipError(SALVA_HIP_E_INVALID, "particle_radius and smoothing_factor must be positive");
    if (p.solver != SALVA_HIP_SOLVER_DFSPH && p.solver != SALVA_HIP_SOLVER_IISPH)
        throw HipError(SALVA_HIP_E_INVALID, "unknown solver kind");
    int ndev = 0;
    hipError_t e = hipGetDeviceCount(&ndev);
    if (e != hipSuccess || ndev == 0)
        throw HipError(SALVA_HIP_E_HIP, "no HIP device available: libsalva_hip has no CPU fallback");
    if (p.device < 0 || p.device >= ndev) throw HipError(SALVA_HIP_E_INVALID, "device ordinal out of range");
    use_device();
    const float h = p.particle_radius * p.smoothing_factor * 2.0f;
    sc = make_sph_consts(h);
    if (p.kernel_density < 0 || p.kernel_density > SALVA_HIP_KERNEL_VISCOSITY || p.kernel_gradient < 0 || p.kernel_gradient > SALVA_HIP_KERNEL_VISCOSITY)
        throw HipError(SALVA_HIP_E_INVALID, "unknown kernel kind");
    sc.kd = p.kernel_density;
    sc.kg = p.kernel_gradient;
    SALVA_HIP_CHECK(hipStreamCreateWithFlags(&stream, hipStreamNonBlocking));
    SALVA_HIP_CHECK(hipStreamCreateWithFlags(&stream2, hipStreamNonBlocking));
    SALVA_HIP_CHECK(hipEventCreateWithFlags(&ev_pre_refresh, hipEventDisableTiming));
    SALVA_HIP_CHECK(hipEventCreateWithFlags(&ev_interior, hipEventDisableTiming));
    SALVA_HIP_CHECK(hipEventCreateWithFlags(&ev_spec_eval, hipEventDisableTiming));
    SALVA_HIP_CHECK(hipEventCreateWithFlags(&ev_spec_apply, hipEventDisableTiming));
    spec_dist_off = getenv("SALVA_HIP_NO_SPEC_DIST") != nullptr;
    overlap_exchange = getenv("SALVA_HIP_NO_OVERLAP") == nullptr;
    spec_off = getenv("SALVA_HIP_SPECULATE") == nullptr || getenv("SALVA_HIP_NO_SPECULATION") != nullptr;
    spec_tight = getenv("SALVA_HIP_SPEC_TIGHT") != nullptr;
    defer_off = getenv("SALVA_HIP_NO_DEFER_LISTS") != nullptr;
    spec_apply_off = getenv("SALVA_HIP_NO_SPEC_APPLY") != nullptr;
    chain_off = getenv("SALVA_HIP_NO_CHAIN") != nullptr;
    pre_off = getenv("SALVA_HIP_NO_PREGRID") != nullptr;
    split_off = getenv("SALVA_HIP_NO_SPLIT") != nullptr;
    classes_off = getenv("SALVA_HIP_NO_CLASSES") != nullptr;
    classes_forced = getenv("SALVA_HIP_CLASSES") != nullptr;
    light_on = getenv("SALVA_HIP_LIGHT") != nullptr;
    ref_off = getenv("SALVA_HIP_FULL_HALO") != nullptr;
    ref_forced = getenv("SALVA_HIP_REF_HALO") != nullptr;
    ref_tight = getenv("SALVA_HIP_REF_TIGHT") != nullptr;
    if (const char* e = getenv("SALVA_HIP_SPLIT_S")) split_forced = (uint32_t)std::max(atoi(e), 1);
    no_planes = getenv("SALVA_HIP_NO_PLANES") != nullptr;
    two_mass_off = getenv("SALVA_HIP_NO_TWO_MASS") != nullptr;
    if (const char* e = getenv("SALVA_HIP_MAX_MASSES")) max_masses = (uint32_t)std::min(std::max(atoi(e), 2), 4);
    fold_off = getenv("SALVA_HIP_NO_FOLD") != nullptr;
    if (const char* e = getenv("SALVA_HIP_FOLD_CELLS")) {
        const long v = atol(e);
        if (v >= 8 && v <= (1 << 20) && (v & (v - 1)) == 0) fold_forced = (uint32_t)v;
    }
    tile_trace = getenv("SALVA_HIP_TILE_TRACE") != nullptr;
    no_fused_div = getenv("SALVA_HIP_NO_FUSED_DIV") != nullptr;
    if (const char* e = getenv("SALVA_HIP_RADIX_SORT")) sort_mode = atoi(e) != 0 ? 1 : 0;
    if (const char* e = getenv("SALVA_HIP_DS_LEVEL")) lds.ds_level = (uint32_t)std::max(0, atoi(e));
#ifdef SALVA_HIP_DIAG
    if (const char* e = getenv("SALVA_HIP_SCHED")) sched_mode = atoi(e);
#endif
    if (const char* e = getenv("SALVA_HIP_LIST_CAP0")) { cap_ff = std::max<uint32_t>(LIST_REGS, ((uint32_t)atoi(e) + 3u) & ~3u); trust_cap0 = true; }
    {
        int cus = 0;
        if (hipDeviceGetAttribute(&cus, hipDeviceAttributeMultiprocessorCount, p.device) == hipSuccess && cus > 0) num_cus = cus;
    }
    SALVA_HIP_CHECK(hipHostMalloc((void**)&h_rb, sizeof(Readback), hipHostMallocDefault));
    memset(h_rb, 0, sizeof(Readback));
    SALVA_HIP_CHECK(hipHostMalloc((void**)&h_ctl, 2 * NUM_SOLVES * sizeof(SolveCtl), hipHostMallocDefault));
    memset(h_ctl, 0, 2 * NUM_SOLVES * sizeof(SolveCtl));
    SALVA_HIP_CHECK(hipHostMalloc((void**)&h_pub, NUM_SOLVES * sizeof(SolveCtl), hipHostMallocMapped | hipHostMallocCoherent));
    memset(h_pub, 0, NUM_SOLVES * sizeof(SolveCtl));
    SALVA_HIP_CHECK(hipHostMalloc((void**)&h_hostpub, sizeof(HostPub), hipHostMallocMapped | hipHostMallocCoherent));
    memset(h_hostpub, 0, sizeof(HostPub));
    d_ctl.ensure(NUM_SOLVES);
    d_rb.ensure(1);
    d_flags.p = &d_rb.p->flags;
    SALVA_HIP_CHECK(hipMemset(d_rb.p, 0, sizeof(Readback)));
    {
        mass_slots.ensure(2 * MASS_SLOTS);
        SALVA_HIP_CHECK(hipMemset(mass_slots.p, 0, 2 * MASS_SLOTS * sizeof(uint32_t)));
    }
    d_counters.ensure(4);
    for (auto& e2 : ev) SALVA_HIP_CHECK(hipEventCreate(&e2));
    for (auto& e2 : evc) SALVA_HIP_CHECK(hipEventCreate(&e2));
    SALVA_HIP_CHECK(hipEventCreateWithFlags(&ev_sync, hipEventDisableTiming));
}

World::~World() {
    (void)hipSetDevice(prm.device);
    if (stream) { (void)hipStreamSynchronize(stream); (void)hipStreamDestroy(stream); }
    if (stream2) { (void)hipStreamSynchronize(stream2); (void)hipStreamDestroy(stream2); }
    if (dl_stream) { (void)hipStreamSynchronize(dl_stream); (void)hipStreamDestroy(dl_stream); }
    if (ev_dl_ready) (void)hipEventDestroy(ev_dl_ready);
    if (ev_dl_done) (void)hipEventDestroy(ev_dl_done);
    for (float* p : h_dl) if (p) (void)hipHostFree(p);
    for (hipEvent_t e : dist_ev) if (e) (void)hipEventDestroy(e);
    if (ev_pre_refresh) (void)hipEventDestroy(ev_pre_refresh);
    if (ev_interior) (void)hipEventDestroy(ev_interior);
    if (ev_spec_eval) (void)hipEventDestroy(ev_spec_eval);
    if (ev_spec_apply) (void)hipEventDestroy(ev_spec_apply);
    if (h_rb) (void)hipHostFree(h_rb);
    if (h_ctl) (void)hipHostFree(h_ctl);
    if (h_pub) (void)hipHostFree(h_pub);
    if (h_hostpub) (void)hipHostFree(h_hostpub);
    for (auto& e : ev) if (e) (void)hipEventDestroy(e);
    for (auto& e : evc) if (e) (void)hipEventDestroy(e);
    if (ev_sync) (void)hipEventDestroy(ev_sync);
}

void World::use_device() const { SALVA_HIP_CHECK(hipSetDevice(prm.device)); }

uint64_t World::fluid_offset(uint32_t slot) const {
    uint64_t o = 0;
    for (uint32_t s = 0; s < slot; ++s) o += fluids[s].n;
    return o;
}
uint64_t World::boundary_offset(uint32_t slot) const {
    uint64_t o = 0;
    for (uint32_t s = 0; s < slot; ++s) o += bounds[s].n;
    return o;
}
// ... 398 lines not shown
}

void World::upload_tables() {
    if (!tables_dirty) return;
    lists_checked = trust_cap0;
    const uint32_t nm = (uint32_t)std::max<size_t>(fluids.size(), 1), nbm = (uint32_t)std::max<size_t>(bounds.size(), 1);
    std::vector<float> r0(nm, 1000.0f);
    std::vector<uint32_t> counts(nm, 0);
    std::vector<uint8_t> ff(nm * nm, 1), fb(nm * nbm, 1), bb(nbm * nbm, 1), bw(nbm, 0);
    any_wants_forces = false;
    for (uint32_t a = 0; a < fluids.size(); ++a) {
        r0[a] = fluids[a].density0;
        counts[a] = (uint32_t)fluids[a].n;
        for (uint32_t b = 0; b < fluids.size(); ++b)
            ff[a * nm + b] = (a == b) || groups_test(fluids[a].memberships, fluids[a].filter, fluids[b].memberships, fluids[b].filter);
        for (uint32_t b = 0; b < bounds.size(); ++b)
            fb[a * nbm + b] = groups_test(fluids[a].memberships, fluids[a].filter, bounds[b].memberships, bounds[b].filter);
    }
    for (uint32_t a = 0; a < bounds.size(); ++a) {
        bw[a] = bounds[a].wants_forces ? 1 : 0;
        any_wants_forces |= bounds[a].wants_forces;
        for (uint32_t b = 0; b < bounds.size(); ++b)
            bb[a * nbm + b] = (a == b) || groups_test(bounds[a].memberships, bounds[a].filter, bounds[b].memberships, bounds[b].filter);
    }
    rho0_tab.ensure(nm); model_counts.ensure(nm); ff_ok.ensure(nm * nm); fb_ok.ensure(nm * nbm); bb_ok.ensure(nbm * nbm); bwants.ensure(nbm);
    SALVA_HIP_CHECK(hipMemcpyAsync(rho0_tab.p, r0.data(), nm * sizeof(float), hipMemcpyHostToDevice, stream));
    if (comm && dist_started && global_counts.size() == nm) counts = global_counts;
    SALVA_HIP_CHECK(hipMemcpyAsync(model_counts.p, counts.data(), nm * sizeof(uint32_t), hipMemcpyHostToDevice, stream));
    SALVA_HIP_CHECK(hipMemcpyAsync(ff_ok.p, ff.data(), ff.size(), hipMemcpyHostToDevice, stream));
    SALVA_HIP_CHECK(hipMemcpyAsync(fb_ok.p, fb.data(), fb.size(), hipMemcpyHostToDevice, stream));
    SALVA_HIP_CHECK(hipMemcpyAsync(bb_ok.p, bb.data(), bb.size(), hipMemcpyHostToDevice, stream));
    SALVA_HIP_CHECK(hipMemcpyAsync(bwants.p, bw.data(), bw.size(), hipMemcpyHostToDevice, stream));
    SALVA_HIP_CHECK(hipStreamSynchronize(stream));
    tables_dirty = false;
    b_dirty = true;
}

float World::bforce_scale() const {
    const float r = prm.particle_radius;
    return std::exp2f(36.0f - std::ceil(std::log2(1000.0f * r * r * r)));
}

StepCtx World::make_ctx() {
    StepCtx c{};
    if (any_wants_forces && bforce_fx_n != nb) {
        bforce_fx.ensure(3 * (size_t)std::max<uint32_t>(nb, 1u), stream, false, 1.2f);
        SALVA_HIP_CHECK(hipMemsetAsync(bforce_fx.p, 0, 3 * (size_t)std::max<uint32_t>(nb, 1u) * sizeof(unsigned long long), stream));
        bforce_fx_n = nb;
    }
    c.sc = sc;
    {
        uint32_t lg = 1u;
        while (lg < 7u && (16u << lg) <= nlaunch) ++lg;
        c.xcd = lg;
    }
    c.n = n;
    c.posm = posm[cur].p; c.vel = vel[cur].p; c.dv = dv[cur].p; c.acc = acc.p; c.w = w.p; c.normal = normal.p;
    c.model = model[cur].p; c.perm = perm[cur].p; c.gtag = comm ? gtag[cur].p : nullptr;
    c.rho = rho.p; c.alpha = alpha.p; c.kappa = kappa.p; c.kappa2 = kappa2.p; c.rho_star = rho_star.p; c.aii = aii.p;
    c.dii = dii.p; c.dijpj = dijpj.p; c.iisph_q = iisph_q.p; c.iisph_pr = iisph_pr.p; c.posmr = posmr.p;
    c.nff = nff.p; c.nfb = nfb.p;
    c.nbr_ff = nbr_ff.p; c.nbr_fb = nbr_fb.p; c.cap_ff = cap_ff; c.cap_fb = cap_fb;
    c.slice_near = slice_near.p;
    c.tile_off = G().tile_off.p; c.halo_src = halo_src.p; c.bhalo_src = bhalo_src.p;
    c.halo_stride = halo_stride; c.bhalo_stride = bhalo_stride;
    c.ntiles = (uint32_t)gf.ntiles();
    c.split_s = split_s_cur;
    c.slot_order = (class_ntiny || class_nlight) ? slot_order.p : nullptr; c.slot_base = 0u; c.ntiny = class_ntiny; c.nlight = class_nlight;
    c.tile_ids = G().tile_ids.p; c.tile_rank = G().tile_rank.p; c.nlaunch = nlaunch; c.slot_desc = G().slot_desc.p; c.slot_info = slot_info.p;
    c.spec = spec_mode ? 1u : 0u; c.halo_cap = halo_cap; c.bhalo_cap = bhalo_cap; c.nslices_cap = nslices_cap;
    c.halo_len = halo_len; c.bhalo_len = bhalo_len;
    c.gf = gf.device(G().cell_start_f.p);
    c.stale_keys = has_dynamic_sampling() ? G().keys[1].p : nullptr;
    c.nb = nb;
    c.bposv = bposv.p; c.bvel = bvel.p; c.bperm = bperm.p;
    c.bforce = any_wants_forces ? bforce.p : nullptr;
    c.bforce_fx = any_wants_forces ? bforce_fx.p : nullptr;
    c.bforce_scale = bforce_scale();
    c.bwants = bwants.p;
    c.gb = gb.device(cell_start_b.p);
    c.nmodels = (uint32_t)std::max<size_t>(fluids.size(), 1);
    c.nbmodels = (uint32_t)std::max<size_t>(bounds.size(), 1);
    c.mass_uniform = mass_uniform;
    c.two_mass = two_mass ? 1u : 0u;
    c.nmass = two_mass ? nmass : 0u; c.cmask = mass_cmask;
    for (int k = 0; k < 4; ++k) c.class_mass[k] = mass_classes[k];
    c.tile_mass_bits = two_mass ? tile_mass_bits.p : nullptr;
    c.tile_massb_bits = two_mass ? tile_massb_bits.p : nullptr;
    c.tile_masscd_bits = (two_mass && nmass > 2u) ? tile_masscd_bits.p : nullptr;
    c.nffb = two_mass ? nffb.p : nullptr;
    c.nffc = (two_mass && nmass > 2u) ? nffc.p : nullptr;
    c.bvel_zero = 1u;
    for (const BoundarySlot& b : bounds) if (b.n && (!b.vel_zero || b.sampling || b.dyn_kind)) c.bvel_zero = 0u;
    c.rho0_tab = rho0_tab.p; c.rho0_single = fluids.empty() ? 1000.0f : fluids[0].density0; c.ff_ok = ff_ok.p; c.fb_ok = fb_ok.p; c.bb_ok = bb_ok.p;
    c.partials = partials.p;
    c.spec_k = -1; c.spec_ring = spec_ring.p; c.spec_pub = nullptr; c.model_counts = model_counts.p; c.w2 = w2.p;
    c.flags = d_flags.p;
    c.min_neighbors_for_divergence = 20;
    c.phase = 0;
    c.ghost_lo_cx = (comm && comm->has_lo()) ? slab_lo - 1 : INT32_MIN;
    c.ghost_hi_cx = (comm && comm->has_hi()) ? slab_hi + 1 : INT32_MAX;
    return c;
}

struct FoldRule { double budget, target; uint32_t min_period[3]; bool axis[3]; };
static void dims_from_bbox(const int32_t* bb, GridDims& g, const FoldRule* fold = nullptr) {
    static const int T[3] = {TX, TY, TZ};
    int64_t cells[3];
    for (int a = 0; a < 3; ++a) {
        if (bb[a] > bb[3 + a]) throw HipError(SALVA_HIP_E_CAPACITY, "empty cell bounding box");
        const int64_t extent = (int64_t)bb[3 + a] - (int64_t)bb[a] + 1;
        if (extent > (1 << 30)) throw HipError(SALVA_HIP_E_CAPACITY, "cell bounding box too large");
        g.o[a] = bb[a];
        g.nt[a] = (int)((extent + T[a] - 1) / T[a]);
        g.mask[a] = 0xffffffffu;
        cells[a] = (int64_t)g.nt[a] * T[a];
    }
    if (fold && (double)cells[0] * (double)cells[1] * (double)cells[2] > fold->budget) {
        for (;;) {
            if ((double)cells[0] * (double)cells[1] * (double)cells[2] <= fold->target) break;
            int best = -1;
            int64_t best_p = 0;
            for (int a = 0; a < 3; ++a) {
                int64_t p = 1;
                while (p * 2 < cells[a]) p *= 2;
                if (!fold->axis[a] || p < (int64_t)fold->min_period[a] || p >= cells[a]) continue;
                if (best < 0 || cells[a] > cells[best]) { best = a; best_p = p; }
            }
            if (best < 0) break;
            cells[best] = best_p;
            g.nt[best] = (int)(best_p / T[best]);
            g.mask[best] = (uint32_t)best_p - 1u;
        }
    }
    const double nc = (double)cells[0] * (double)cells[1] * (double)cells[2];
    if (nc >= 4.0e9) throw HipError(SALVA_HIP_E_CAPACITY, "dense cell table would exceed 2^32 cells; particles are too spread out");
    static const double budget_gib = [] {
        const char* e = getenv("SALVA_HIP_CELL_TABLE_GIB");
        const double v = e ? atof(e) : 8.0;
        return v > 0.0 ? v : 8.0;
    }();
    const double gib = (nc * 4.0 + nc / TCELLS * 8.0) / (1024.0 * 1024.0 * 1024.0);
    if (gib > budget_gib) {
        char msg[512];
        snprintf(msg, sizeof msg,
                 "the cell table over the particles' bounding box (%d x %d x %d tiles of %dx%dx%d cells) would take %.1f GiB, over the "
                 "%.1f GiB budget: particles are too spread out for the dense grid — delete strays (salva_hip_particles_intersecting_aabb "
                 "+ salva_hip_delete_particles) or raise SALVA_HIP_CELL_TABLE_GIB",
                 g.nt[0], g.nt[1], g.nt[2], TX, TY, TZ, gib, budget_gib);
        throw HipError(SALVA_HIP_E_CAPACITY, msg);
    }
}

void World::build_boundary_grid() {
    if (!b_dirty) return;
    ncontacts_bb = 0;
    if (nb == 0) { b_dirty = false; return; }
    bbox_partials.ensure(6 * std::max<size_t>(bbox_blocks(nb), 1024));
    launch_bbox(bst_pos.p, nb, sc.h, bbox_partials.p, d_rb.p->bbbox, d_flags.p, stream);
    SALVA_HIP_CHECK(hipMemcpyAsync(h_rb->bbbox, d_rb.p->bbbox, sizeof(int32_t) * 6, hipMemcpyDeviceToHost, stream));
    SALVA_HIP_CHECK(hipStreamSynchronize(stream));
    dims_from_bbox(h_rb->bbbox, gb);
    const size_t nc = gb.ncells();
    bkeys[0].ensure(nb); bkeys[1].ensure(nb); bidx[0].ensure(nb); bidx[1].ensure(nb);
    bposv.ensure(nb); bvel.ensure(nb); bperm.ensure(nb); cell_start_b.ensure(nc + 1);
    TileGrid gv = gb.device(nullptr);
// ... 907 lines not shown
    check_mass = have_grid ? pre.check_mass : !(mass_known && mass_uniform == 0.0f);
    if (!have_grid) {
        TileGrid gv = gf.device(nullptr);
        const bool counting = ncf + 1 < 0x7fffffffull && (sort_mode == 0 || (sort_mode < 0 && ncf <= 16ull * n + (1ull << 20)));
        if (counting) {
            G().cell_rank.ensure(n, stream, false, 1.1f);
            SALVA_HIP_CHECK(hipMemsetAsync(G().cell_start_f.p, 0, (ncf + 1) * sizeof(uint32_t), stream));
        }
        launch_cell_keys(posm[cur].p, n, sc.h, gv, G().keys[0].p, G().idx[0].p, d_flags.p, check_mass ? mass_slots.p : nullptr,
                         counting ? G().cell_start_f.p : nullptr, counting ? G().cell_rank.p : nullptr, stream);
        if (has_dyn) {
            if (timers) wait_stream();
            const auto t1 = std::chrono::steady_clock::now();
            run_dynamic_sampling();
            dcs_ms = std::chrono::duration<double, std::milli>(std::chrono::steady_clock::now() - t1).count();
        }
        if (counting) {
            const size_t tb = cell_sort_temp_bytes((uint32_t)ncf);
            ensure_cub_temp(tb);
            cell_sort(cub_temp.p, tb, n, (uint32_t)ncf, G().keys[0].p, G().cell_rank.p, G().cell_start_f.p, G().keys[1].p, G().idx[0].p, G().idx[1].p, stream);
        } else {
            const int end_bit = bits_for(ncf);
            const size_t tb = sort_pairs_temp_bytes(n, end_bit);
            ensure_cub_temp(tb);
            sort_pairs(cub_temp.p, tb, G().keys[0].p, G().keys[1].p, G().idx[0].p, G().idx[1].p, n, end_bit, stream);
            launch_cell_start(G().keys[1].p, n, (uint32_t)ncf, G().cell_start_f.p, stream);
        }
    }
    auto reorder = [&]() {
        launch_reorder_fluid(n, G().idx[1].p, arrays(cur), arrays(cur ^ 1), w.p, stream);
        cur ^= 1;
        if (timers) SALVA_HIP_CHECK(hipEventRecord(evc[0], stream));
        if (acc_user && !comm) launch_gather_f4(n, perm[cur].p, st_acc.p, acc.p, stream);
        if (comm) dist_build_lists();
    };
    build_boundary_grid();
    if (timers) SALVA_HIP_CHECK(hipEventRecord(evc[1], stream));

    nlaunch = 0;
    spec_mode = false; halo_cap = bhalo_cap = 0xffffffffu; nslices_cap = 0xffffffffu; halo_len = bhalo_len = ~0ull;
    c = make_ctx();
    TileAcc tt{};
    uint32_t nslices = 0;
    {
        const size_t tb = std::max(scan_tiles_temp_bytes(nslots_bound + 1), scan_temp_bytes(ntiles + 1));
        ensure_cub_temp(tb);
        if (!have_grid) {
        launch_tile_slots(gf.device(G().cell_start_f.p), ntiles, G().tile_flags.p, G().tile_rank.p, G().tile_ids.p, cub_temp.p, tb, stream, nullptr, split_s_cur);
        if (nslots_bound == 0) SALVA_HIP_CHECK(hipMemsetAsync(G().tile_cnt.p, 0, sizeof(TileAcc), stream));
        launch_tile_count(c, nslots_bound, G().tile_cnt.p, G().slot_desc.p, stream);
        scan_tiles(cub_temp.p, tb, G().tile_cnt.p, G().tile_off.p, nslots_bound + 1, stream);
        }
        if (spec) {
            const TileAcc& l = pred_tt;
            tt = l;
            const uint32_t m = spec_tight ? 0u : 1u;
            tt.nonempty = std::min<uint32_t>(nslots_bound, l.nonempty + m * std::max<uint32_t>(16u, l.nonempty / 16u));
            tt.max_s = (l.max_s + m * std::max<uint32_t>(32u, l.max_s / 16u) + m * 63u) & ~(m * 63u);
            tt.max_sb = nb ? ((l.max_sb + m * std::max<uint32_t>(32u, l.max_sb / 8u) + m * 63u) & ~(m * 63u)) : 0u;
            tt.nsl = std::min<uint32_t>(n / WAVE + nslots_bound + 1, l.nsl + m * std::max<uint32_t>(64u, l.nsl / 32u));
            tt.s = l.s + m * (l.s / 8 + 4096); tt.sb = l.sb + m * (l.sb / 4 + 4096);
            TileLds probe; probe.max_halo_fluid = tt.max_s; probe.max_halo_boundary = tt.max_sb;
            if (probe.bytes(52, 32, 6) > 160u * 1024u || tt.max_s >= 65536u || tt.max_sb >= 65536u) spec = false;
        }
        if (!spec) {
            const uint32_t seq = have_grid ? pre.seq : publish_enqueue(G().tile_off.p + nslots_bound, false, false);
            reorder();
            publish_wait(seq, true, false, false);
            tt = h_rb->tile_total;
            if (check_mass) {
                float m;
                memcpy(&m, &h_rb->mass_mm[0], sizeof(m));
                mass_uniform = (h_rb->mass_mm[0] == h_rb->mass_mm[1] && m > 0.0f && std::isfinite(m) && !no_planes) ? m : 0.0f;
                mass_known = true;
            }
        } else {
            reorder();
        }
        nlaunch = tt.nonempty;
        lds.max_halo_fluid = tt.max_s;
        lds.max_halo_boundary = tt.max_sb;
        lds.max_sum = spec ? 0u : tt.max_sum;
        lds.max_raw = spec ? 0u : tt.max_raw;
        if (tile_trace)
            fprintf(stderr, "salva_hip tiles: nonempty %u max_s %u max_sb %u max_sum %u max_raw %u heavy %u light %u tiny %u split_s %u mass_uniform %g | chained %llu breaks %llu pregrid %llu dropped %llu | fold %u %u %u\n",
                    tt.nonempty, tt.max_s, tt.max_sb, tt.max_sum, tt.max_raw, tt.heavy, tt.nlight, tt.ntiny, split_s_cur, (double)mass_uniform,
                    (unsigned long long)chain_steps, (unsigned long long)chain_breaks, (unsigned long long)pre_adopted, (unsigned long long)pre_dropped,
                    gf.mask[0] + 1u, gf.mask[1] + 1u, gf.mask[2] + 1u);
        if (!spec) {
            if (!split_on) split_on = tt.heavy > 0u && (uint64_t)tt.heavy * 5u <= tt.nonempty;
            else if ((uint64_t)tt.heavy * 2u > tt.nonempty) split_on = false;
        }
        {
#ifndef SALVA_TILE_WAVES_CAP
#define SALVA_TILE_WAVES_CAP 8
#endif
            static_assert(SALVA_TILE_WAVES_CAP <= TILE_MAX_WAVES, "the launch bounds are written for TILE_MAX_WAVES");
            const uint32_t avg = (n + tt.nonempty - 1) / std::max<uint32_t>(tt.nonempty, 1u);
            const uint32_t lo = (HCELLS + WAVE - 1) / WAVE, hi = std::min<uint32_t>(std::max<uint32_t>(tt.max_nsl, lo), (uint32_t)(SALVA_TILE_WAVES_CAP));
#ifdef SALVA_TILE_WAVES_PLAIN_AVERAGE
            const uint32_t weighted = 0u;
#else
            const uint32_t weighted = tt.nsl ? (uint32_t)((double)tt.wsl / (double)tt.nsl + 0.5) : 0u;
#endif
            lds.threads = WAVE * std::min<uint32_t>(std::max<uint32_t>(std::max<uint32_t>((avg + WAVE - 1) / WAVE, weighted), lo), hi);
        }
#ifdef SALVA_HIP_DIAG
        if (const char* e = getenv("SALVA_HIP_TILE_THREADS")) lds.threads = (uint32_t)atoi(e);
#endif
        if (gf.folded() && !fold_locked && !spec) {
            TileLds probe; probe.max_halo_fluid = tt.max_s; probe.max_halo_boundary = tt.max_sb; probe.max_sum = tt.max_sum;
            if (tt.max_s >= 65536u || tt.max_sb >= 65536u || probe.bytes(52, 32, 6) > 160u * 1024u) {
                ++fold_relax;
                throw FoldRetry{};
            }
        }
        if (lds.max_halo_fluid >= 65536u || lds.max_halo_boundary >= 65536u)
            throw HipError(SALVA_HIP_E_CAPACITY, "more than 65535 particles in one tile halo");
        if (tt.nsl > ns_cap) throw HipError(SALVA_HIP_E_HIP, "internal error: slice count exceeds its bound");
        {
            const uint64_t st_f = (lds.max_halo_fluid + 63u) & ~63u, st_b = nb ? ((lds.max_halo_boundary + 63u) & ~63u) : 0u;
            const uint64_t strided = (uint64_t)nlaunch * (st_f + st_b), compact = tt.s + tt.sb;
            const bool use = strided <= 3 * compact + (1u << 20) && !getenv("SALVA_HIP_COMPACT_HALO");
            halo_stride = use ? (uint32_t)st_f : 0u;
            bhalo_stride = use ? (uint32_t)st_b : 0u;
        }
#ifdef SALVA_HIP_DIAG
        {
            pipe.enabled = halo_stride > 0 && !getenv("SALVA_HIP_NO_PIPELINE");
            pipe.scap = halo_stride;
            pipe.sbcap = bhalo_stride;
            pipe.num_cus = (uint32_t)num_cus;
            pipe.nlaunch = nlaunch;
            uint32_t waves = std::min<uint32_t>(std::max<uint32_t>(tt.max_nsl, 4u), (uint32_t)PIPE_MAX_WAVES);
            if (const char* e = getenv("SALVA_HIP_PIPE_WAVES")) waves = std::min<uint32_t>(std::max(atoi(e), 1), PIPE_MAX_WAVES);
            pipe.threads = waves * WAVE;
        }
#endif
        const size_t need_f = halo_stride ? (size_t)nlaunch * halo_stride : (size_t)tt.s;
        const size_t need_b = halo_stride ? (size_t)nlaunch * bhalo_stride : (size_t)tt.sb;
        halo_src.ensure(need_f ? need_f : 1, stream, false, 1.2f);
        bhalo_src.ensure(need_b ? need_b : 1, stream, false, 1.2f);
        nslices = tt.nsl;
        if (spec) {
            spec_mode = true;
            halo_cap = lds.max_halo_fluid; bhalo_cap = lds.max_halo_boundary; nslices_cap = nslices;
            halo_len = need_f; bhalo_len = need_b;
        }
        class_ntiny = class_nlight = 0u;
        if (!spec && !classes_off) {
            if (tt.ntiny > 0u && tt.ntiny < tt.nonempty && (classes_forced || tt.ntiny >= 512u)) class_ntiny = tt.ntiny;
            const bool beyond = tt.max_s > P3_DS_THREE || tt.max_raw > P2_DS_THREE || tt.max_sum > FIXED_DS_SMALL;
            const uint32_t nfull = tt.nonempty - tt.nlight - tt.ntiny;
            if (tt.nlight > 0u && nfull > 0u && (classes_forced || (light_on && beyond && tt.nlight >= 256u))) class_nlight = tt.nlight;
            if (class_nlight && !class_ntiny) class_nlight += tt.ntiny;
        }
        if (class_ntiny || class_nlight) slot_order.ensure(nlaunch, stream, false, 1.5f);
        if (class_nlight) ++counters.light_class_passes;
        if (class_ntiny) ++counters.sparse_class_passes;
        auto fill_tables = [&](bool again) {
            const uint32_t keep_t = class_ntiny, keep_l = class_nlight;
            class_ntiny = class_nlight = 0u;
            c = make_ctx();
            if (again) scan_tiles(cub_temp.p, tb, G().tile_cnt.p, G().tile_off.p, nslots_bound + 1, stream);
            launch_tile_halo_fill(c, halo_src.p, bhalo_src.p, slot_info.p, stream, (keep_t || keep_l) ? slot_order.p : nullptr, keep_l, keep_t);
            class_ntiny = keep_t; class_nlight = keep_l;
        };
        fill_tables(false);
        c = make_ctx();

        const bool beyond3 = tt.max_s > P3_DS_THREE || tt.max_raw > P2_DS_THREE || tt.max_sum > FIXED_DS_SMALL;
        const bool ref_step = !ref_off && !spec && n > 0 && halo_stride > 0u && c.nmodels <= 32u && c.nbmodels <= 32u && (ref_forced || beyond3);
        RefBuild refb{halo_src.p, slot_info.p, G().tile_off.p, RefCaps{0xffffffffu, 0xffffffffu, 0xffffffffu}, d_rb.p->max_ref};
        ref_bounded = false;
        if (ref_step && defer_lists && ref_pred_valid && ref_pred_n == n) {
            auto bound = [&](uint32_t pred, uint32_t full, uint32_t layout) {
                if (ref_tight) return std::min(pred - pred / 8u, full);
                uint32_t b = pred + std::max<uint32_t>(96u, pred / 8u);
                if (b > layout && pred + 8u <= layout) b = layout;
                return std::min(b, full);
            };
            refb.cap.s = bound(ref_pred[0], tt.max_s, P3_DS_THREE);
            refb.cap.raw = std::max(bound(ref_pred[1], tt.max_raw, P2_DS_THREE), tt.max_sb);
            refb.cap.sum = std::max(bound(ref_pred[2], tt.max_sum, FIXED_DS_SMALL), tt.max_sb);
            ref_bounded = true;
        }

        for (int nattempt = 0;; ++nattempt) {
            if (nattempt > 0 && ref_step) { fill_tables(true); }
            const bool r1 = nbr_ff.ensure((size_t)nslices * cap_ff * WAVE + 1, stream, false, 1.1f);
            const bool r2 = nbr_fb.ensure(nb ? (size_t)nslices * cap_fb * WAVE + 1 : 1, stream, false, 1.1f);
            slice_near.ensure((size_t)nslices + 1, stream, false, 1.1f);
// ... 1037 lines not shown
void World::get_boundary_particles(uint32_t slot, float* positions, float* velocities) {
    use_device();
    if (slot >= bounds.size()) throw HipError(SALVA_HIP_E_INVALID, "boundary slot out of range");
    const uint64_t nn = bounds[slot].n, off = boundary_offset(slot);
    if (nn == 0) return;
    scratch_f.ensure(3 * nn, stream, false, 1.1f);
    for (int k = 0; k < 2; ++k) {
        float* out = k == 0 ? positions : velocities;
        if (!out) continue;
        k_unpack_xyz<<<nblk(nn), BLOCK, 0, stream>>>((uint32_t)nn, (k == 0 ? bst_pos.p : bst_vel.p) + off, scratch_f.p);
        SALVA_HIP_CHECK(hipMemcpyAsync(out, scratch_f.p, 3 * nn * sizeof(float), hipMemcpyDeviceToHost, stream));
        SALVA_HIP_CHECK(hipStreamSynchronize(stream));
    }
}

void World::get_boundary_wrench(uint32_t slot, const float point[3], float force[3], float torque[3]) {
    use_device();
    if (slot >= bounds.size()) throw HipError(SALVA_HIP_E_INVALID, "boundary slot out of range");
    const BoundarySlot& b = bounds[slot];
    for (int k = 0; k < 3; ++k) force[k] = torque[k] = 0.0f;
    if (!b.n || !b.wants_forces) return;
    const uint64_t off = boundary_offset(slot);
    const uint32_t nblocks = (uint32_t)std::min<uint64_t>(nblk(b.n), 256);
    wrench_partial.ensure((size_t)256 * 6);
    k_boundary_wrench<<<nblocks, BLOCK, 0, stream>>>((uint32_t)b.n, bst_pos.p + off, bforce.p + off, point[0], point[1], point[2], wrench_partial.p);
    SALVA_HIP_CHECK(hipGetLastError());
    std::vector<double> h((size_t)nblocks * 6);
    SALVA_HIP_CHECK(hipMemcpyAsync(h.data(), wrench_partial.p, h.size() * sizeof(double), hipMemcpyDeviceToHost, stream));
    SALVA_HIP_CHECK(hipStreamSynchronize(stream));
    double acc[6] = {0, 0, 0, 0, 0, 0};
    for (uint32_t k = 0; k < nblocks; ++k)
        for (int j = 0; j < 6; ++j) acc[j] += h[(size_t)k * 6 + j];
    for (int k = 0; k < 3; ++k) { force[k] = (float)acc[k]; torque[k] = (float)acc[3 + k]; }
}

void World::clear_boundary_forces(uint32_t slot) {
    use_device();
    if (slot >= bounds.size()) throw HipError(SALVA_HIP_E_INVALID, "boundary slot out of range");
    const uint64_t nn = bounds[slot].n, off = boundary_offset(slot);
    if (nn) {
        SALVA_HIP_CHECK(hipMemsetAsync(bforce.p + off, 0, nn * sizeof(float4), stream));
        SALVA_HIP_CHECK(hipStreamSynchronize(stream));
    }
}

uint64_t World::device_bytes() const {
    uint64_t b = 0;
    auto add = [&](size_t x) { b += x; };
    add(st_pos.bytes()); add(st_vel.bytes()); add(st_dv.bytes()); add(st_acc.bytes()); add(st_model.bytes());
    for (int k = 0; k < 2; ++k) {
        add(posm[k].bytes()); add(vel[k].bytes()); add(dv[k].bytes()); add(model[k].bytes()); add(perm[k].bytes());
        for (const GridTabs& t : gtab) { add(t.keys[k].bytes()); add(t.idx[k].bytes()); }
        add(bkeys[k].bytes()); add(bidx[k].bytes());
    }
    add(acc.bytes()); add(w.bytes()); add(normal.bytes()); add(dii.bytes()); add(dijpj.bytes()); add(iisph_q.bytes()); add(iisph_pr.bytes()); add(posmr.bytes()); add(w2.bytes());
    add(rho.bytes()); add(alpha.bytes()); add(kappa.bytes()); add(kappa2.bytes()); add(rho_star.bytes()); add(aii.bytes());
    add(visc_beta.bytes()); add(visc_target.bytes()); add(visc_u0.bytes()); add(visc_u1.bytes()); add(visc_va.bytes()); add(he_colors.bytes()); add(he_gradcs.bytes());
    add(nff.bytes()); add(nfb.bytes()); add(gtab[0].cell_start_f.bytes()); add(gtab[1].cell_start_f.bytes()); add(halo_src.bytes()); add(bhalo_src.bytes());
    add(nbr_ff.bytes()); add(nbr_fb.bytes()); add(slice_near.bytes()); add(cub_temp.bytes()); add(scratch_f.bytes());
    add(scratch_f4.bytes()); add(bst_pos.bytes()); add(bst_vel.bytes()); add(bposv.bytes()); add(bvel.bytes());
    add(bforce.bytes()); add(bperm.bytes()); add(cell_start_b.bytes()); add(partials.bytes());
    return b;
}

float World::time_pred_density(int reps) {
    use_device();
    if (!have_last_ctx || !sorted_valid || n == 0) throw HipError(SALVA_HIP_E_INVALID, "no completed step to time");
    if (reps < 1) reps = 1;
#ifdef SALVA_HIP_DIAG
    if (getenv("SALVA_HIP_TILE_TIMING")) tile_timing_report();
#endif
    flags_clean = false;
    launch_pred_density(last_ctx, lds, last_dt, stream);
    SALVA_HIP_CHECK(hipEventRecord(ev[0], stream));
    for (int r = 0; r < reps; ++r) launch_pred_density(last_ctx, lds, last_dt, stream);
    SALVA_HIP_CHECK(hipEventRecord(ev[1], stream));
    SALVA_HIP_CHECK(hipStreamSynchronize(stream));
    float ms = 0.0f;
    SALVA_HIP_CHECK(hipEventElapsedTime(&ms, ev[0], ev[1]));
    return ms * 1000.0f / (float)reps;
}


void World::tile_tables(uint32_t slot, uint32_t* info, uint32_t* halo_row, uint32_t cap_row, uint32_t* counts, uint32_t cap_counts, uint32_t* entries,
                        uint32_t cap_entries) {
    use_device();
    if (!have_last_ctx || !sorted_valid || n == 0) throw HipError(SALVA_HIP_E_INVALID, "no completed step to look at");
    const StepCtx& c = last_ctx;
    if (slot >= c.nlaunch) throw HipError(SALVA_HIP_E_INVALID, "no such tile slot");
    SALVA_HIP_CHECK(hipStreamSynchronize(stream));
    TileAcc a[2];
    uint4 desc;
    SALVA_HIP_CHECK(hipMemcpy(a, c.tile_off + slot, sizeof(a), hipMemcpyDeviceToHost));
    SALVA_HIP_CHECK(hipMemcpy(&desc, c.slot_desc + slot, sizeof(desc), hipMemcpyDeviceToHost));
    const uint32_t S = (uint32_t)(a[1].s - a[0].s), SB = (uint32_t)(a[1].sb - a[0].sb), own_n = desc.z - desc.y;
    const uint64_t hoff = c.halo_stride ? (uint64_t)slot * c.halo_stride : a[0].s;
    memset(info, 0, 16 * sizeof(uint32_t));
    info[0] = c.nlaunch; info[1] = desc.y; info[2] = desc.z; info[3] = S; info[4] = SB;
    info[5] = lds.max_halo_fluid; info[6] = lds.raw_slots(); info[7] = lds.sum_slots(); info[8] = lds_full.max_halo_fluid;
    info[9] = ref_last ? 1u : 0u; info[10] = (uint32_t)ref_passes; info[11] = (uint32_t)ref_misses;
    if (halo_row && cap_row && S)
        SALVA_HIP_CHECK(hipMemcpy(halo_row, c.halo_src + hoff, (size_t)std::min(S, cap_row) * sizeof(uint32_t), hipMemcpyDeviceToHost));
    if (!own_n) return;
    std::vector<uint32_t> cnt(own_n);
    SALVA_HIP_CHECK(hipMemcpy(cnt.data(), c.nff + desc.y, (size_t)own_n * sizeof(uint32_t), hipMemcpyDeviceToHost));
    if (counts) memcpy(counts, cnt.data(), (size_t)std::min(own_n, cap_counts) * sizeof(uint32_t));
    if (!entries || !cap_entries) return;
    const uint32_t nsl = (own_n + WAVE - 1) / WAVE;
    std::vector<uint32_t> blk((size_t)nsl * c.cap_ff * WAVE);
    SALVA_HIP_CHECK(hipMemcpy(blk.data(), c.nbr_ff + (size_t)a[0].nsl * c.cap_ff * WAVE, blk.size() * sizeof(uint32_t), hipMemcpyDeviceToHost));
    uint32_t o = 0;
    for (uint32_t k = 0; k < own_n; ++k) {
        const uint32_t* p = blk.data() + (size_t)(k / WAVE) * c.cap_ff * WAVE + 4u * (k % WAVE);
        for (uint32_t e = 0; e < cnt[k] && o < cap_entries; ++e) {
            const uint32_t d = p[ellq(e >> 1)];
            entries[o++] = (e & 1u) ? (d >> 16) : (d & 0xffffu);
        }
    }
    info[12] = o;
}

float World::time_kernel(int kernel, int reps) {
    use_device();
    if (!have_last_ctx || !sorted_valid || n == 0) throw HipError(SALVA_HIP_E_INVALID, "no completed step to time");
    if (kernel == 0) return time_pred_density(reps);
    if (reps < 1) reps = 1;
    const bool iisph = prm.solver == SALVA_HIP_SOLVER_IISPH;
    if (kernel == 4 && comm) throw HipError(SALVA_HIP_E_INVALID, "not available in a multi-GPU run");
    if ((kernel == 2 || kernel == 3) && !iisph) throw HipError(SALVA_HIP_E_INVALID, "an IISPH kernel needs an IISPH world");
    if (kernel == 1 && iisph) throw HipError(SALVA_HIP_E_INVALID, "k_divergence needs a DFSPH world");
    StepCtx cd = last_ctx;
    cd.ctl = nullptr;
    flags_clean = false;
    if (kernel == 6) {
        if (iisph) throw HipError(SALVA_HIP_E_INVALID, "k_divergence_apply needs a DFSPH world");
        w2.ensure(n, stream, false, 1.1f);
        SALVA_HIP_CHECK(hipMemcpyAsync(w2.p, w.p, (size_t)n * sizeof(float4), hipMemcpyDeviceToDevice, stream));
        cd.w = w2.p; cd.w2 = w2.p; cd.spec_k = -1; cd.bforce = nullptr;
    }
    ElasticState* el = nullptr;
    uint32_t el_slot = 0, el_force = 0;
    DevBuf<float4> acc_copy;
    DevBuf<float> el_sig, el_F;
    bool el_swapped = false;
    struct Unswap {
        ElasticState*& e; DevBuf<float>& s; DevBuf<float>& f; bool& on;
        ~Unswap() { if (on) { std::swap(e->sig.p, s.p); std::swap(e->sig.cap, s.cap); std::swap(e->F.p, f.p); std::swap(e->F.cap, f.cap); } }
    } unswap{el, el_sig, el_F, el_swapped};
    if (kernel == 7 || kernel == 8) {
        for (uint32_t f = 0; f < fluids.size() && !el; ++f)
            for (uint32_t k = 0; k < fluids[f].forces.size() && !el; ++k)
                if (fluids[f].forces[k].kind == SALVA_HIP_FORCE_BECKER2009 && k < fluids[f].elastic.size() && fluids[f].elastic[k] &&
                    fluids[f].elastic[k]->list_valid && fluids[f].elastic[k]->n0 == fluids[f].n) {
                    el = fluids[f].elastic[k].get(); el_slot = f; el_force = k;
                }
        if (!el) throw HipError(SALVA_HIP_E_INVALID, "no Becker2009Elasticity entry has run");
        if (comm) throw HipError(SALVA_HIP_E_INVALID, "not available in a multi-GPU run");
        cd.gate = nullptr;
        acc_copy.ensure(n);
        SALVA_HIP_CHECK(hipMemcpyAsync(acc_copy.p, cd.acc, (size_t)n * sizeof(float4), hipMemcpyDeviceToDevice, stream));
        SALVA_HIP_CHECK(hipMemcpyAsync(el->rot_new.p, el->rot.p, 9 * el->n0 * sizeof(float), hipMemcpyDeviceToDevice, stream));
        if (kernel == 7) {
            el_sig.ensure(6 * el->n0); el_F.ensure(9 * el->n0);
            std::swap(el->sig.p, el_sig.p); std::swap(el->sig.cap, el_sig.cap);
            std::swap(el->F.p, el_F.p); std::swap(el->F.cap, el_F.cap);
            el_swapped = true;
        }
    }
    const ElasticParams el_p = el ? elastic_params(fluids[el_slot].forces[el_force].p) : ElasticParams{};
    const uint32_t el_off = el ? (uint32_t)fluid_offset(el_slot) : 0u;
    auto launch = [&]() {
        switch (kernel) {
            case 7: launch_elastic_rot_stress(cd, *el, el_p, stream); break;
            case 8: launch_elastic_forces(cd, el_off, *el, el_p, acc_copy.p, stream); break;
            case 1: launch_divergence(cd, lds, stream); break;
            case 6: launch_divergence_apply(cd, lds, inv_dt_prev, stream); break;
            case 2: launch_iisph_next_pressure(cd, lds, last_dt, 0.5f, kappa.p, kappa2.p, stream); break;
            case 3: launch_iisph_dij_pj(cd, lds, last_dt, kappa.p, stream); break;
            case 4:
                cd.stale_keys = G().keys[1].p;
                if (ref_last) {
                    StepCtx cf = cd;
                    cf.slot_order = nullptr; cf.ntiny = cf.nlight = 0u; cf.slot_base = 0u;
// ... 28 lines not shown
```

Measured before the change: 409.6 million.

## Split tail-slice neighbor sums across idle waves in divergence kernels

```diff
diff --git a/salva_amd/csrc/device_types.h b/salva_amd/csrc/device_types.h
--- a/salva_amd/csrc/device_types.h
+++ b/salva_amd/csrc/device_types.h
@@ -87,6 +87,7 @@
     uint32_t bhalo_stride;
     uint32_t ntiles;
     uint32_t split_s;
+    uint32_t tail_split;
     const uint32_t* tile_ids;
     const uint4* slot_desc;
     const uint4* slot_info;
diff --git a/salva_amd/csrc/dfsph.hip b/salva_amd/csrc/dfsph.hip
--- a/salva_amd/csrc/dfsph.hip
+++ b/salva_amd/csrc/dfsph.hip
@@ -1,3 +1,4 @@
+#include <type_traits>
 #include <climits>
 
 #include "bbox.h"
@@ -398,7 +399,7 @@
     TileErrC E;
     E.init(reinterpret_cast<float*>(t.pool + t.pool_used), c);
     Tile::staged_barrier();
-    t.for_own_pre(own0, load_own, [&](const Own& o, uint32_t i, uint32_t gs, bool active) {
+    auto body = [&](const Own& o, uint32_t i, uint32_t gs, bool active, auto halves, float hlo, float hhi) {
         const uint32_t nqu = slice_list_dwords(o.cnt, active);
         const bool near = slice_is_near(c, o.near);
         float err = 0.0f;
@@ -411,6 +412,9 @@
                 const float4 pi = make_float4(o.px, o.py, o.pz, 0.0f), wi = make_float4(o.ux, o.uy, o.uz, 0.0f);
                 if ((TWO && t.massb != 0.0f) && !near) {
                     div += pair_sum_velocity_divergence_p3_two(c, gs, nqu, o.lh, pi, wi, dist8, o.cnt - o.nb2, t.mass, t.massb);
+                } else if constexpr (decltype(halves)::value) {
+                    div += near ? pair_sum_velocity_divergence_exact_p3(c, i, gs, pi, wi, dist8, t.mass)
+                                : (hlo + hhi) * c.sc.gscale * t.mass;
                 } else {
                     div += near ? pair_sum_velocity_divergence_exact_p3(c, i, gs, pi, wi, dist8, t.mass)
                                 : pair_sum_velocity_divergence_p3(c, gs, nqu, o.lh, pi, wi, dist8, t.mass);
@@ -434,7 +438,36 @@
             err = div / rho0;
         }
         E.add(c, err, mi, active && !is_ghost(c, i));
-    });
+    };
+    const uint32_t extra = TWO ? 0u : t.tail_extra(c);
+    auto whole = [&](const Own& o, uint32_t i, uint32_t gs, bool active) { body(o, i, gs, active, std::false_type{}, 0.0f, 0.0f); };
+    {
+        const uint32_t s = threadIdx.x / WAVE, i = t.own_begin + threadIdx.x;
+        if (s < (t.own_end - t.own_begin + WAVE - 1) / WAVE) whole(own0, i, t.slice_base + s, i < t.own_end);
+    }
+    if (TWO == 0 && extra) {
+        const uint32_t lane = threadIdx.x & (WAVE - 1), nw = blockDim.x / WAVE;
+        const uint32_t wv = (uint32_t)__builtin_amdgcn_readfirstlane((int)(threadIdx.x / WAVE));
+        float* const part = reinterpret_cast<float*>(t.pool + t.pool_used + TileErrC::bytes(c));
+        const bool owner = wv < extra, helper = wv + extra >= nw;
+        const uint32_t e = owner ? wv : nw - 1u - wv;
+        const uint32_t i = t.own_begin + (nw + e) * WAVE + lane, gs = t.slice_base + nw + e;
+        const bool active = (owner || helper) && i < t.own_end;
+        Own o = own0;
+        float half = 0.0f;
+        if (owner || helper) {
+            o = load_own(active ? i : t.own_begin, gs);
+            const uint32_t nqu = slice_list_dwords(o.cnt, active);
+            if (!slice_is_near(c, o.near) && active && o.cnt + o.cntb >= c.min_neighbors_for_divergence)
+                half = pair_half_velocity_divergence_p3(c, gs, nqu, o.lh, make_float4(o.px, o.py, o.pz, 0.0f), make_float4(o.ux, o.uy, o.uz, 0.0f),
+                                                        dist8, helper ? 16u : 0u);
+            if (helper) part[e * WAVE + lane] = half;
+        }
+        __syncthreads();
+        if (owner) body(o, i, gs, active, std::true_type{}, half, part[e * WAVE + lane]);
+    } else {
+        t.for_own_rest(load_own, whole);
+    }
     E.finish(c, t.slot);
 }
 template <uint32_t DS>
@@ -541,7 +574,7 @@
     const uint32_t dist8 = p2_dist8<DS>(t);
     t.stage_p2(c, static_cast<const float4*>(c.posm), static_cast<const float*>(c.kappa), dist8);
     Tile::staged_barrier();
-    t.for_own_pre(own0, load_own, [&](const Own& o, uint32_t i, uint32_t gs, bool active) {
+    auto body = [&](const Own& o, uint32_t i, uint32_t gs, bool active, auto halves, const float (&hlo)[3], const float* hhi) {
         const uint32_t nqu = slice_list_dwords(o.cnt, active);
         const bool near = slice_is_near(c, o.near);
         if (!active) return;
@@ -552,6 +585,10 @@
             pair_sum_gradient_p2_two(c, gs, nqu, o.lh, pi, dist8, o.cnt - o.nb2, t.mass, t.massb, [&](float ka, float kb) { return f2{ki + ka, ki + kb}; }, sx, sy, sz);
         } else {
             if (near) pair_sum_gradient_exact_p2(c, i, gs, pi, dist8, t.mass, [&](float kj) { return ki + kj; }, sx, sy, sz);
+            else if constexpr (decltype(halves)::value) {
+                const float f = c.sc.gscale * t.mass;
+                sx = (hlo[0] + hhi[0]) * f; sy = (hlo[1] + hhi[WAVE]) * f; sz = (hlo[2] + hhi[2 * WAVE]) * f;
+            }
             else pair_sum_gradient_p2(c, gs, nqu, o.lh, pi, dist8, t.mass, [&](float ka, float kb) { return f2{ki + ka, ki + kb}; }, sx, sy, sz);
             if ((TWO && t.massb != 0.0f) && o.nb2) {
                 float bx, by, bz;
@@ -592,7 +629,39 @@
             }
         });
         wout[i] = d;
-    });
+    };
+    const float none[3] = {0.0f, 0.0f, 0.0f};
+    const uint32_t extra = TWO ? 0u : t.tail_extra(c);
+    auto whole = [&](const Own& o, uint32_t i, uint32_t gs, bool active) { body(o, i, gs, active, std::false_type{}, none, nullptr); };
+    {
+        const uint32_t s = threadIdx.x / WAVE, i = t.own_begin + threadIdx.x;
+        if (s < (t.own_end - t.own_begin + WAVE - 1) / WAVE) whole(own0, i, t.slice_base + s, i < t.own_end);
+    }
+    if (TWO == 0 && extra) {
+        const uint32_t lane = threadIdx.x & (WAVE - 1), nw = blockDim.x / WAVE;
+        const uint32_t wv = (uint32_t)__builtin_amdgcn_readfirstlane((int)(threadIdx.x / WAVE));
+        float* const part = reinterpret_cast<float*>(t.pool + ((t.pool_used + 15u) & ~15u));
+        const bool owner = wv < extra, helper = wv + extra >= nw;
+        const uint32_t e = owner ? wv : nw - 1u - wv;
+        const uint32_t i = t.own_begin + (nw + e) * WAVE + lane, gs = t.slice_base + nw + e;
+        const bool active = (owner || helper) && i < t.own_end;
+        Own o = own0;
+        float half[3] = {0.0f, 0.0f, 0.0f};
+        float* const mine = part + e * (3u * WAVE) + lane;
+        if (owner || helper) {
+            o = load_own(active ? i : t.own_begin, gs);
+            const uint32_t nqu = slice_list_dwords(o.cnt, active);
+            const float ki = o.ki;
+            if (!slice_is_near(c, o.near) && active)
+                pair_half_gradient_p2(c, gs, nqu, o.lh, make_float4(o.px, o.py, o.pz, 0.0f), dist8, helper ? 16u : 0u,
+                                      [&](float ka, float kb) { return f2{ki + ka, ki + kb}; }, half[0], half[1], half[2]);
+            if (helper) { mine[0] = half[0]; mine[WAVE] = half[1]; mine[2 * WAVE] = half[2]; }
+        }
+        __syncthreads();
+        if (owner) body(o, i, gs, active, std::true_type{}, half, mine);
+    } else {
+        t.for_own_rest(load_own, whole);
+    }
 }
 template <uint32_t DS>
 __global__ SALVA_P2_BOUNDS(DS) void k_divergence_apply_p2(StepCtx c, float inv_dt_prev) { k_divergence_apply_p2_body<DS, 0>(c, inv_dt_prev); }
diff --git a/salva_amd/csrc/pairs.h b/salva_amd/csrc/pairs.h
--- a/salva_amd/csrc/pairs.h
+++ b/salva_amd/csrc/pairs.h
@@ -75,6 +75,23 @@
     });
     return (acc2.x + acc2.y) * c.sc.gscale * mass;
 }
+__device__ __forceinline__ float pair_half_velocity_divergence_p3(const StepCtx& c, uint32_t gs, uint32_t nqu, const ListRegs& lh, const float4& pi,
+                                                                  const float4& wi, uint32_t dist8, uint32_t sh) {
+    float acc = 0.0f;
+    const f2 tiny = {1.0e-30f, 1.0e-30f};
+    for_each_ff_half<2>(c, gs, nqu, lh, sh, [&](uint32_t o) { return load_p3(o, dist8); }, [&](const RecP3& A, const RecP3& B, bool two) { SALVA_PAIR_MATH
+        const f2 dx = {pi.x - A.xy.x, pi.x - B.xy.x}, dy = {pi.y - A.xy.y, pi.y - B.xy.y}, dz = {pi.z - A.zu.x, pi.z - B.zu.x};
+        f2 r2 = dz * dz + tiny;
+        r2 = dy * dy + r2;
+        r2 = dx * dx + r2;
+        const f2 g = kernel_gfac2(r2, c.sc);
+        const f2 ux = {wi.x - A.zu.y, wi.x - B.zu.y}, uy = {wi.y - A.vw.x, wi.y - B.vw.x}, uz = {wi.z - A.vw.y, wi.z - B.vw.y};
+        const f2 s = ux * dx + uy * dy + uz * dz;
+        acc = __builtin_fmaf(s.x, g.x, acc);
+        if (two) acc = __builtin_fmaf(s.y, g.y, acc);
+    });
+    return acc;
+}
 __device__ __forceinline__ float pair_sum_velocity_divergence_p3_two(const StepCtx& c, uint32_t gs, uint32_t nqu, const ListRegs& lh, const float4& pi,
                                                                      const float4& wi, uint32_t dist8, uint32_t na, float ma, float mb) {
     f2 acc2 = {0.0f, 0.0f};
@@ -144,6 +161,23 @@
     sx = (ax.x + ax.y) * f; sy = (ay.x + ay.y) * f; sz = (az.x + az.y) * f;
 }
 template <typename K2>
+__device__ __forceinline__ void pair_half_gradient_p2(const StepCtx& c, uint32_t gs, uint32_t nqu, const ListRegs& lh, const float4& pi,
+                                                      uint32_t dist8, uint32_t sh, K2&& kij2, float& hx, float& hy, float& hz) {
+    float ax = 0.0f, ay = 0.0f, az = 0.0f;
+    const f2 tiny = {1.0e-30f, 1.0e-30f};
+    for_each_ff_half<2>(c, gs, nqu, lh, sh, [&](uint32_t o) { return load_p2(o, dist8); }, [&](const RecP2& A, const RecP2& B, bool two) { SALVA_PAIR_MATH
+        const f2 dx = {pi.x - A.xy.x, pi.x - B.xy.x}, dy = {pi.y - A.xy.y, pi.y - B.xy.y}, dz = {pi.z - A.zk.x, pi.z - B.zk.x};
+        f2 r2 = dz * dz + tiny;
+        r2 = dy * dy + r2;
+        r2 = dx * dx + r2;
+        const f2 g = kernel_gfac2(r2, c.sc);
+        const f2 coeff = kij2(A.zk.y, B.zk.y) * g;
+        ax = __builtin_fmaf(dx.x, coeff.x, ax); ay = __builtin_fmaf(dy.x, coeff.x, ay); az = __builtin_fmaf(dz.x, coeff.x, az);
+        if (two) { ax = __builtin_fmaf(dx.y, coeff.y, ax); ay = __builtin_fmaf(dy.y, coeff.y, ay); az = __builtin_fmaf(dz.y, coeff.y, az); }
+    });
+    hx = ax; hy = ay; hz = az;
+}
+template <typename K2>
 __device__ __forceinline__ void pair_sum_gradient_p2_two(const StepCtx& c, uint32_t gs, uint32_t nqu, const ListRegs& lh, const float4& pi,
                                                          uint32_t dist8, uint32_t na, float ma, float mb, K2&& kij2, float& sx, float& sy, float& sz) {
     f2 ax = {0.0f, 0.0f}, ay = {0.0f, 0.0f}, az = {0.0f, 0.0f};
@@ -192,7 +226,7 @@
 static inline uint32_t p2_bytes(const TileLds& L, uint32_t ds) {
     const uint32_t n = L.raw_slots();
     const uint32_t dist8 = ds ? ds * 8u : ((n * 8u + 15u) & ~15u);
-    return dist8 + n * 8u + 32u;
+    return dist8 + n * 8u + 32u + (L.tail_split ? TILE_TAIL_P2_BYTES : 0u);
 }
 
 template <typename K2>
@@ -263,7 +297,8 @@
     const uint32_t by_maxima = ((L.max_halo_fluid * 8u + 15u) & ~15u) + bb * L.max_halo_boundary;
     const uint32_t by_raw = ((L.raw_slots() * 8u + 15u) & ~15u) + (bb - 8u) * L.max_halo_boundary;
     static const uint32_t pad = getenv("SALVA_HIP_P3_PAD") ? (uint32_t)atoi(getenv("SALVA_HIP_P3_PAD")) : 0u;
-    return 2u * dist8 + (by_raw < by_maxima ? by_raw : by_maxima) + ((TILE_MAX_WAVES * nmodels * 4u + 15u) & ~15u) + 32u + pad;
+    return 2u * dist8 + (by_raw < by_maxima ? by_raw : by_maxima) + ((TILE_MAX_WAVES * nmodels * 4u + 15u) & ~15u) + 32u + pad +
+           (L.tail_split ? TILE_TAIL_P3_BYTES : 0u);
 }
 static inline uint32_t pick_ds_p2(uint32_t n, uint32_t level) {
     const uint32_t ds[4] = {P2_DS_THREE, P3_DS_TWO, P3_DS_ONE, 0u};
diff --git a/salva_amd/csrc/tile.h b/salva_amd/csrc/tile.h
--- a/salva_amd/csrc/tile.h
+++ b/salva_amd/csrc/tile.h
@@ -25,6 +25,7 @@
     uint32_t max_sum = 0;
     uint32_t max_raw = 0;
     uint32_t ds_level = 0;
+    uint32_t tail_split = 1;
     uint32_t raw_slots() const { return max_raw ? max_raw : max_halo_fluid + max_halo_boundary; }
     uint32_t sum_slots() const {
         const uint32_t worst = ((max_halo_fluid + 63u) & ~63u) + max_halo_boundary;
@@ -58,6 +59,8 @@
 __host__ __device__ inline uint32_t tile_part_code(uint32_t ux0, uint32_t len) { return ux0 | ((len - 1u) << 2); }
 constexpr uint32_t TILE_SPLIT_S = P3_DS_THREE;
 constexpr uint32_t TILE_TINY_S = 192, TILE_TINY_SB = 64, TILE_TINY_THREADS = 64;
+constexpr uint32_t TILE_TAIL_MAX = 2;
+constexpr uint32_t TILE_TAIL_P3_BYTES = TILE_TAIL_MAX * 64u * 4u, TILE_TAIL_P2_BYTES = 3u * TILE_TAIL_P3_BYTES;
 constexpr uint32_t TILE_ERR_BYTES = 12u * 32u * 4u;
 
 #ifdef __HIPCC__
@@ -497,19 +500,29 @@
     template <typename Pre, typename LoadOwn, typename Body>
     __device__ __forceinline__ void for_own_pre(const Pre& pre0, LoadOwn&& load_own, Body&& body) const {
         const uint32_t nsl = (own_end - own_begin + WAVE - 1) / WAVE;
-        const uint32_t lane = threadIdx.x & (WAVE - 1), nw = blockDim.x / WAVE;
-        uint32_t s = threadIdx.x / WAVE;
+        const uint32_t lane = threadIdx.x & (WAVE - 1), s = threadIdx.x / WAVE;
         if (s < nsl) {
             const uint32_t i = own_begin + s * WAVE + lane;
             body(pre0, i, slice_base + s, i < own_end);
-            s += nw;
-        }
-        for (; s < nsl; s += nw) {
+        }
+        for_own_rest(load_own, body);
+    }
+    template <typename LoadOwn, typename Body>
+    __device__ __forceinline__ void for_own_rest(LoadOwn&& load_own, Body&& body) const {
+        const uint32_t nsl = (own_end - own_begin + WAVE - 1) / WAVE;
+        const uint32_t lane = threadIdx.x & (WAVE - 1), nw = blockDim.x / WAVE;
+        for (uint32_t s = threadIdx.x / WAVE + nw; s < nsl; s += nw) {
             const uint32_t i = own_begin + s * WAVE + lane, gs = slice_base + s;
             const bool active = i < own_end;
-            const Pre p = load_own(active ? i : own_begin, gs);
+            const auto p = load_own(active ? i : own_begin, gs);
             body(p, i, gs, active);
         }
+    }
+
+    __device__ __forceinline__ uint32_t tail_extra(const StepCtx& c) const {
+        const uint32_t nsl = (own_end - own_begin + WAVE - 1) / WAVE, nw = blockDim.x / WAVE;
+        const uint32_t extra = nsl > nw ? nsl - nw : 0u;
+        return (c.tail_split && extra <= TILE_TAIL_MAX && 2u * extra <= nw) ? extra : 0u;
     }
 
     template <typename F>
@@ -806,6 +819,45 @@
         }
     }
 }
+template <int OFF>
+__device__ __forceinline__ uint32_t entry_half(uint32_t a, uint32_t sh) {
+    const uint32_t e = __builtin_amdgcn_ubfe(a, sh, 16u);
+    return OFF == 1 ? e << 4 : OFF == 2 ? e << 3 : e;
+}
+template <int OFF, typename L, typename C2>
+__device__ __forceinline__ void for_each_ff_half(const StepCtx& c, uint32_t gslice, uint32_t nq, const ListRegs& lr, uint32_t sh, L&& load,
+                                                 C2&& compute2) {
+    static_assert(LIST_REGS % 4 == 0, "four dwords per step");
+#pragma unroll
+    for (int k = 0; k < LIST_REGS; k += 4) {
+        if ((uint32_t)(k + 2) < nq) {
+            const bool four = (uint32_t)(k + 3) < nq;
+            const uint32_t a = lr.d[k], b = lr.d[k + 1], e = lr.d[k + 2], f = four ? lr.d[k + 3] : e;
+            const auto d0 = load(entry_half<OFF>(a, sh));
+            const auto d1 = load(entry_half<OFF>(b, sh));
+            const auto d2 = load(entry_half<OFF>(e, sh));
+            const auto d3 = load(entry_half<OFF>(f, sh));
+            compute2(d0, d1, true);
+            compute2(d2, d3, four);
+        } else if ((uint32_t)k < nq) {
+            const bool two = (uint32_t)(k + 1) < nq;
+            const uint32_t a = lr.d[k], b = two ? lr.d[k + 1] : a;
+            const auto d0 = load(entry_half<OFF>(a, sh));
+            const auto d1 = load(entry_half<OFF>(b, sh));
+            compute2(d0, d1, two);
+        }
+    }
+    if (nq > (uint32_t)LIST_REGS) {
+        const uint32_t* __restrict__ p = c.nbr_ff + (size_t)gslice * c.cap_ff * WAVE + 4u * (threadIdx.x & (WAVE - 1));
+        for (uint32_t q = LIST_REGS; q < nq; q += 2) {
+            const bool two = q + 1 < nq;
+            const uint32_t a = p[ellq(q)], b = two ? p[ellq(q + 1)] : a;
+            const auto d0 = load(entry_half<OFF>(a, sh));
+            const auto d1 = load(entry_half<OFF>(b, sh));
+            compute2(d0, d1, two);
+        }
+    }
+}
 constexpr int FB_REGS = 8;
 struct FbRegs { uint32_t d[FB_REGS]; };
 __device__ __forceinline__ FbRegs fb_regs(const StepCtx& c, uint32_t gslice) {
diff --git a/salva_amd/csrc/world.h b/salva_amd/csrc/world.h
--- a/salva_amd/csrc/world.h
+++ b/salva_amd/csrc/world.h
@@ -339,6 +339,8 @@
     uint32_t class_nlight = 0;
     bool classes_off = false, classes_forced = false, light_on = false;
     bool split_off = false;
+    bool tail_off = false;
+    void tail_stats(const uint4* slot_desc, uint32_t nslots, uint32_t waves, uint32_t* out4);
     bool ref_off = false, ref_forced = false;
     bool ref_tight = false;
     bool ref_on_cur = false;
diff --git a/salva_amd/csrc/world.hip b/salva_amd/csrc/world.hip
--- a/salva_amd/csrc/world.hip
+++ b/salva_amd/csrc/world.hip
@@ -138,6 +138,8 @@
     chain_off = getenv("SALVA_HIP_NO_CHAIN") != nullptr;
     pre_off = getenv("SALVA_HIP_NO_PREGRID") != nullptr;
     split_off = getenv("SALVA_HIP_NO_SPLIT") != nullptr;
+    tail_off = getenv("SALVA_HIP_NO_TAIL_SPLIT") != nullptr;
+    lds.tail_split = tail_off ? 0u : 1u;
     classes_off = getenv("SALVA_HIP_NO_CLASSES") != nullptr;
     classes_forced = getenv("SALVA_HIP_CLASSES") != nullptr;
     light_on = getenv("SALVA_HIP_LIGHT") != nullptr;
@@ -702,6 +704,7 @@
     c.nmodels = (uint32_t)std::max<size_t>(fluids.size(), 1);
     c.nbmodels = (uint32_t)std::max<size_t>(bounds.size(), 1);
     c.mass_uniform = mass_uniform;
+    c.tail_split = tail_off ? 0u : 1u;
     c.two_mass = two_mass ? 1u : 0u;
     c.nmass = two_mass ? nmass : 0u; c.cmask = mass_cmask;
     for (int k = 0; k < 4; ++k) c.class_mass[k] = mass_classes[k];
@@ -1775,11 +1778,6 @@
         lds.max_halo_boundary = tt.max_sb;
         lds.max_sum = spec ? 0u : tt.max_sum;
         lds.max_raw = spec ? 0u : tt.max_raw;
-        if (tile_trace)
-            fprintf(stderr, "salva_hip tiles: nonempty %u max_s %u max_sb %u max_sum %u max_raw %u heavy %u light %u tiny %u split_s %u mass_uniform %g | chained %llu breaks %llu pregrid %llu dropped %llu | fold %u %u %u\n",
-                    tt.nonempty, tt.max_s, tt.max_sb, tt.max_sum, tt.max_raw, tt.heavy, tt.nlight, tt.ntiny, split_s_cur, (double)mass_uniform,
-                    (unsigned long long)chain_steps, (unsigned long long)chain_breaks, (unsigned long long)pre_adopted, (unsigned long long)pre_dropped,
-                    gf.mask[0] + 1u, gf.mask[1] + 1u, gf.mask[2] + 1u);
         if (!spec) {
             if (!split_on) split_on = tt.heavy > 0u && (uint64_t)tt.heavy * 5u <= tt.nonempty;
             else if ((uint64_t)tt.heavy * 2u > tt.nonempty) split_on = false;
@@ -1801,6 +1799,15 @@
 #ifdef SALVA_HIP_DIAG
         if (const char* e = getenv("SALVA_HIP_TILE_THREADS")) lds.threads = (uint32_t)atoi(e);
 #endif
+        if (tile_trace) {
+            uint32_t tail[4] = {0, 0, 0, 0};
+            if (!spec) tail_stats(G().slot_desc.p, nlaunch, lds.threads / WAVE, tail);
+            fprintf(stderr, "salva_hip tiles: nonempty %u max_s %u max_sb %u max_sum %u max_raw %u heavy %u light %u tiny %u split_s %u mass_uniform %g | chained %llu breaks %llu pregrid %llu dropped %llu | fold %u %u %u | waves %u max_nsl %u tail_slots %u tail_particles %u tail_shared_slots %u tail_small %u tail_split %u\n",
+                    tt.nonempty, tt.max_s, tt.max_sb, tt.max_sum, tt.max_raw, tt.heavy, tt.nlight, tt.ntiny, split_s_cur, (double)mass_uniform,
+                    (unsigned long long)chain_steps, (unsigned long long)chain_breaks, (unsigned long long)pre_adopted, (unsigned long long)pre_dropped,
+                    gf.mask[0] + 1u, gf.mask[1] + 1u, gf.mask[2] + 1u,
+                    lds.threads / WAVE, tt.max_nsl, tail[0], tail[1], tail[2], tail[3], tail_off ? 0u : 1u);
+        }
         if (gf.folded() && !fold_locked && !spec) {
             TileLds probe; probe.max_halo_fluid = tt.max_s; probe.max_halo_boundary = tt.max_sb; probe.max_sum = tt.max_sum;
             if (tt.max_s >= 65536u || tt.max_sb >= 65536u || probe.bytes(52, 32, 6) > 160u * 1024u) {
@@ -3004,6 +3011,21 @@
 }
 
 
+void World::tail_stats(const uint4* slot_desc, uint32_t nslots, uint32_t waves, uint32_t* out4) {
+    out4[0] = out4[1] = out4[2] = out4[3] = 0u;
+    if (!nslots || !waves) return;
+    std::vector<uint4> desc(nslots);
+    SALVA_HIP_CHECK(hipStreamSynchronize(stream));
+    SALVA_HIP_CHECK(hipMemcpy(desc.data(), slot_desc, (size_t)nslots * sizeof(uint4), hipMemcpyDeviceToHost));
+    for (const uint4& d : desc) {
+        const uint32_t own = d.z - d.y;
+        if (own <= waves * WAVE) continue;
+        const uint32_t beyond = own - waves * WAVE, last = beyond % WAVE, extra = (beyond + WAVE - 1) / WAVE;
+        out4[0] += 1u; out4[1] += beyond; out4[2] += (extra <= TILE_TAIL_MAX && 2u * extra <= waves) ? 1u : 0u;
+        out4[3] += (last && last <= WAVE / 2) ? 1u : 0u;
+    }
+}
+
 void World::tile_tables(uint32_t slot, uint32_t* info, uint32_t* halo_row, uint32_t cap_row, uint32_t* counts, uint32_t cap_counts, uint32_t* entries,
                         uint32_t cap_entries) {
     use_device();
@@ -3021,6 +3043,11 @@
     info[0] = c.nlaunch; info[1] = desc.y; info[2] = desc.z; info[3] = S; info[4] = SB;
     info[5] = lds.max_halo_fluid; info[6] = lds.raw_slots(); info[7] = lds.sum_slots(); info[8] = lds_full.max_halo_fluid;
     info[9] = ref_last ? 1u : 0u; info[10] = (uint32_t)ref_passes; info[11] = (uint32_t)ref_misses;
+    {
+        uint32_t tail[4];
+        tail_stats(c.slot_desc, c.nlaunch, lds.threads / WAVE, tail);
+        info[13] = (lds.threads / WAVE) | (tail_off ? 0u : 1u << 16); info[14] = tail[0]; info[15] = tail[2];
+    }
     if (halo_row && cap_row && S)
         SALVA_HIP_CHECK(hipMemcpy(halo_row, c.halo_src + hoff, (size_t)std::min(S, cap_row) * sizeof(uint32_t), hipMemcpyDeviceToHost));
     if (!own_n) return;
```

Result: no change. 406.3 million (-0.8%).
